# edwardyehuang/iSeg

Hardware: AMD Instinct MI355X
Metric: train_images_per_sec (ConvNeXt-T+ASPP 512x512 crop, fwd+bwd+AdamW, whole job) (higher is better)
Workload: dtype bf16

## Files before the change

### include/iseg_hip.h

```cpp
#ifndef ISEG_HIP_H
#define ISEG_HIP_H

#include <stddef.h>
#include <stdint.h>

#ifdef __cplusplus
extern "C" {
#endif

#ifndef ISEG_HIP_STREAM_T
#define ISEG_HIP_STREAM_T
typedef struct ihipStream_t* iseg_stream_t;
#endif

#define ISEG_STATUS_OK 0
#define ISEG_STATUS_ARG (-1)
#define ISEG_STATUS_HIP (-2)
#define ISEG_STATUS_UNSUPPORTED (-3)
#define ISEG_STATUS_WORKSPACE (-4)

#define ISEG_DTYPE_F32 0
#define ISEG_DTYPE_BF16 1

#define ISEG_ACT_NONE 0
#define ISEG_ACT_RELU 1
#define ISEG_ACT_GELU 2
#define ISEG_ACT_GELU_GRAD 3
#define ISEG_ACT_RELU_GRAD 4
#define ISEG_ACT_MUL_AUX 5
#define ISEG_ACT_SIGMOID 6
#define ISEG_ACT_SWISH 7

int iseg_version(void);
size_t iseg_last_error(char* buf_h, size_t n);

typedef struct iseg_gemm_args {
    const void* A;
    int64_t lda;
    int a_kcontig;
    const void* B;
    int64_t ldb;
    int b_kcontig;
    void* D;
    int64_t ldd;
    int64_t M, N, K;
    int in_dtype, out_dtype;
    const float* bias;
    const float* colscale;
    const float* rowscale;
    int64_t rows_per_group;
    const void* residual;
    int64_t ldr;
    const void* aux;
    int64_t ldaux;
    void* pre_out;
    int64_t ldp;
    int act;
    float alpha;
    int accumulate;
    int split_k;
    int a_act;
    float* colsum_out;
    int colsum_accumulate;
    int defer_reduce;
    int batch, batch_inner;
    int64_t sa_outer, sa_inner, sb_outer, sb_inner, sd_outer, sd_inner;
    int pre_deriv;
    int64_t b_group_rows, b_group_stride;
} iseg_gemm_args;

int iseg_gemm_splits(const iseg_gemm_args* args_h);
int iseg_gemm_slabs(const iseg_gemm_args* args_h);
int iseg_gemm_variant(const iseg_gemm_args* args_h);
size_t iseg_gemm_workspace_bytes(const iseg_gemm_args* args_h);
int iseg_gemm(const iseg_gemm_args* args_h, void* ws, size_t ws_bytes, iseg_stream_t stream);
int iseg_gemm_reduce(const iseg_gemm_args* args_h, void* ws, size_t ws_bytes, iseg_stream_t stream);
int iseg_gemm_tn_pair_splits(const iseg_gemm_args* g0, const iseg_gemm_args* g1);
int iseg_gemm_tn_pair(const iseg_gemm_args* g0, void* ws0, size_t ws0_bytes, const iseg_gemm_args* g1, void* ws1, size_t ws1_bytes,
                      iseg_stream_t stream);

int iseg_layernorm_fwd(const void* x, const float* gamma, const float* beta, void* y, float* mean, float* rstd, int64_t rows,
                       int C, float eps, int dtype, iseg_stream_t stream);
size_t iseg_layernorm_bwd_workspace_bytes(int64_t rows, int C);
int iseg_layernorm_bwd(const void* dy, const void* x, const float* gamma, const float* mean, const float* rstd, void* dx,
                       const void* dx_add, float* dgamma, float* dbeta, int accumulate_param_grads, int64_t rows, int C,
                       int dtype, void* ws, size_t ws_bytes, iseg_stream_t stream);
int iseg_layernorm_post_fwd(const void* x, const float* gamma, const float* beta, const float* colscale, const float* rowscale,
                            int64_t rows_per_group, const void* residual, void* y, float* mean, float* rstd, int64_t rows, int C, float eps,
                            int dtype, iseg_stream_t stream);
int iseg_layernorm_post_bwd(const void* dy, const void* x, const float* gamma, const float* beta, const float* colscale, const float* rowscale,
                            int64_t rows_per_group, const float* mean, const float* rstd, void* dx, float* dgamma, float* dbeta,
                            float* dcolscale, int64_t rows, int C, int dtype, void* ws, size_t ws_bytes, iseg_stream_t stream);
int iseg_layernorm_gather_fwd(const void* x, const int32_t* src_index, const float* gamma, const float* beta, void* y, float* mean,
                              float* rstd, int64_t rows_out, int C, float eps, int dtype, iseg_stream_t stream);
int iseg_layernorm_gather_bwd(const void* dy, const int32_t* dy_index, const void* x, const float* gamma, const float* mean,
                              const float* rstd, void* dx, const void* dx_add, float* dgamma, float* dbeta, int accumulate_param_grads,
                              int64_t rows, int C, int dtype, void* ws, size_t ws_bytes, iseg_stream_t stream);

int iseg_dwconv2d_fwd(const void* x, const float* w, const float* bias, const void* add, void* y, int N, int H, int W, int C,
                      int K, int dil, int pad_t, int pad_l, int flip, int dtype, iseg_stream_t stream);
int iseg_dwconv2d7_mfma(const void* x, const float* w, const float* bias, const void* add, void* y, int N, int H, int W, int C, int pad_t,
                        int pad_l, int flip, iseg_stream_t stream);
size_t iseg_dwconv2d_bwd_weight_workspace_bytes(int N, int H, int W, int C, int K);
int iseg_dwconv2d_bwd_weight(const void* x, const void* dy, float* dw, float* db, int accumulate, int N, int H, int W, int C,
                             int K, int dil, int pad_t, int pad_l, int dtype, void* ws, size_t ws_bytes, iseg_stream_t stream);

int iseg_dwconv2d_strided_fwd(const void* x, const float* w, const float* bias, void* y, int N, int H, int W, int C, int K, int stride, int dil,
                              int pad_t, int pad_l, int Ho, int Wo, int dtype, iseg_stream_t stream);
int iseg_dwconv2d_strided_bwd_data(const void* dy, const float* w, void* dx, int N, int H, int W, int C, int K, int stride, int dil, int pad_t,
                                   int pad_l, int Ho, int Wo, int dtype, iseg_stream_t stream);
size_t iseg_dwconv2d_strided_bwd_weight_workspace_bytes(int N, int Ho, int Wo, int C, int K);
int iseg_dwconv2d_strided_bwd_weight(const void* x, const void* dy, float* dw, float* db, int accumulate, int N, int H, int W, int C, int K,
                                     int stride, int dil, int pad_t, int pad_l, int Ho, int Wo, int dtype, void* ws, size_t ws_bytes,
                                     iseg_stream_t stream);

size_t iseg_bn_workspace_bytes(int64_t rows, int C);
int iseg_bn_stats(const void* x, int64_t ldx, float* packed, int64_t rows, int C, int dtype, void* ws, size_t ws_bytes,
                  iseg_stream_t stream);
int iseg_bn_finalize(const float* packed, int C, float eps, float momentum, float* mean, float* rstd, float* moving_mean,
                     float* moving_var, iseg_stream_t stream);
int iseg_bn_apply_fwd(const void* x, int64_t ldx, const float* mean, const float* rstd, const float* gamma, const float* beta,
                      void* y, int64_t ldy, int64_t rows, int C, int relu, int dtype, iseg_stream_t stream);
int iseg_bn_apply_fwd_packed(const void* x, int64_t ldx, const float* packed, float eps, float momentum, const float* gamma, const float* beta,
                             float* mean, float* rstd, float* moving_mean, float* moving_var, void* y, int64_t ldy, int64_t rows, int C,
                             int relu, int dtype, iseg_stream_t stream);
int iseg_bn_bwd_reduce(const void* dy, int64_t lddy, const void* x, int64_t ldx, const void* y, int64_t ldy, const float* mean,
                       const float* rstd, float* sums, int64_t rows, int C, int relu, int dtype, void* ws, size_t ws_bytes,
                       iseg_stream_t stream);
int iseg_bn_bwd_apply(const void* dy, int64_t lddy, const void* x, int64_t ldx, const void* y, int64_t ldy, const float* mean,
                      const float* rstd, const float* gamma, const float* sums, float inv_n, void* dx, int64_t lddx, int64_t rows,
                      int C, int relu, int dtype, iseg_stream_t stream);
int iseg_bn_bwd_apply_acc(const void* dy, int64_t lddy, const void* x, int64_t ldx, const void* y, int64_t ldy, const float* mean,
                          const float* rstd, const float* gamma, const float* sums, float inv_n, void* dx, int64_t lddx, float* dgamma,
                          float* dbeta, int64_t rows, int C, int relu, int dtype, iseg_stream_t stream);
int iseg_bn_bwd_reduce_remask(const void* dy, int64_t lddy, const void* x, int64_t ldx, const float* mean, const float* rstd,
                              const float* gamma, const float* beta, float* sums, int64_t rows, int C, int dtype, void* ws, size_t ws_bytes,
                              iseg_stream_t stream);
int iseg_bn_bwd_apply_remask(const void* dy, int64_t lddy, const void* x, int64_t ldx, const float* mean, const float* rstd,
                             const float* gamma, const float* beta, const float* sums, float inv_n, void* dx, int64_t lddx, float* dgamma,
                             float* dbeta, int64_t rows, int C, int dtype, iseg_stream_t stream);
int iseg_bn_relu_upsample_add(const void* z, const float* mean, const float* rstd, const float* gamma, const float* beta, const void* x,
                              void* out, int N, int Hi, int Wi, int Ho, int Wo, int C, int dtype, iseg_stream_t stream);
int iseg_rsqrt_eps(const float* var, float eps, float* out, int n, iseg_stream_t stream);

int iseg_mbconv_supported(int N, int HW, int C, int Cse);
size_t iseg_mbconv_partials_bytes(int N, int HW, int C, int backward);
size_t iseg_se_excite_bwd_workspace_bytes(int N, int C, int Cse);
int iseg_bn_swish_se_squeeze(const void* x, const float* mean, const float* rstd, const float* gamma, const float* beta, float* partials,
                             size_t partials_bytes, int N, int HW, int C, int dtype, iseg_stream_t stream);
int iseg_se_excite_fwd(const float* partials, int N, int HW, int C, int Cse, const float* W1, const float* b1, const float* W2, const float* b2,
                       float* m, float* hpre, float* g, iseg_stream_t stream);
int iseg_bn_swish_gate_fwd(const void* x, const float* mean, const float* rstd, const float* gamma, const float* beta, const float* g, void* out,
                           int N, int HW, int C, int dtype, iseg_stream_t stream);
int iseg_bn_swish_gate_bwd_reduce(const void* dO, const void* x, const float* mean, const float* rstd, const float* gamma, const float* beta,
                                  float* partials, size_t partials_bytes, int N, int HW, int C, int dtype, iseg_stream_t stream);
int iseg_se_excite_bwd(const float* partials, int N, int HW, int C, int Cse, const float* W1, const float* W2, const float* m, const float* hpre,
                       const float* g, float* dW1, float* db1, float* dW2, float* db2, int accumulate, float* dmh, float* sums, void* ws,
                       size_t ws_bytes, iseg_stream_t stream);
int iseg_bn_swish_gate_bwd_apply(const void* dO, const void* x, const float* mean, const float* rstd, const float* gamma, const float* beta,
                                 const float* g, const float* dmh, const float* sums, float inv_n, int train, void* dx, float* dgamma,
                                 float* dbeta, int N, int HW, int C, int dtype, iseg_stream_t stream);

int iseg_sepconv_supported(int N, int H, int W, int C, int stride, int dil, int dtype);
size_t iseg_relu_dwconv3_stats_workspace_bytes(int N, int H, int W, int C, int stride, int dil);
int iseg_relu_dwconv3_stats(const void* x, const float* w, void* z, float* packed, int N, int H, int W, int C, int stride, int dil, int dtype,
                            void* ws, size_t ws_bytes, iseg_stream_t stream);
int iseg_sepconv_fold(const float* W, const float* mean, const float* rstd, const float* gamma, const float* beta, void* Wt, void* Wn, float* bias,
                      int Cin, int Cout, int dtype, iseg_stream_t stream);
int iseg_sepconv_fold_bwd(const float* G, const float* S, const float* W, const float* mean, const float* rstd, const float* gamma,
                          const float* beta, float* dW, float* sums, float* dgamma, float* dbeta, int Cin, int Cout, iseg_stream_t stream);
size_t iseg_bnfold_dwconv3_relu_bwd_workspace_bytes(int N, int H, int W, int C, int stride, int dil);
int iseg_bnfold_dwconv3_relu_bwd(const void* D, const void* z, const void* x, const float* w, const float* mean, const float* rstd,
                                 const float* gamma, const float* sums, float inv_n, int train, void* dx, float* dw, int N, int H, int W, int C,
                                 int stride, int dil, int dtype, void* ws, size_t ws_bytes, iseg_stream_t stream);

int iseg_resblock_tail_supported(int C, int stride, int dtype);
size_t iseg_resblock_tail_workspace_bytes(int N, int H, int W, int C, int stride, int bn0);
int iseg_resblock_tail_fwd(const void* z2, const float* mean2, const float* rstd2, const float* gamma2, const float* beta2, const void* sc,
                           const float* mean0, const float* rstd0, const float* gamma0, const float* beta0, void* out, int N, int H, int W, int C,
                           int stride, int dtype, iseg_stream_t stream);
int iseg_resblock_tail_bwd_reduce(const void* dout, const void* out, const void* z2, const float* mean2, const float* rstd2, const void* z0,
                                  const float* mean0, const float* rstd0, float* sums, int N, int H, int W, int C, int stride, int dtype, void* ws,
                                  size_t ws_bytes, iseg_stream_t stream);
int iseg_resblock_tail_bwd_apply(const void* dout, const void* out, const void* z2, const float* mean2, const float* rstd2, const float* gamma2,
                                 const void* z0, const float* mean0, const float* rstd0, const float* gamma0, const float* sums, float inv_n2,
                                 float inv_n0, int train, void* dz2, void* dsc, float* dgamma2, float* dbeta2, float* dgamma0, float* dbeta0,
                                 int N, int H, int W, int C, int stride, int dtype, iseg_stream_t stream);

typedef void* iseg_comm_t;
int iseg_comm_unique_id(void* id128);
int iseg_comm_init(iseg_comm_t* comm, int world_size, int rank, const void* id128);
int iseg_allreduce_sum(iseg_comm_t comm, void* buf, size_t count, int dtype, iseg_stream_t stream);
int iseg_comm_destroy(iseg_comm_t comm);

int iseg_deferred_begin(void* grad_base, size_t grad_bytes, void* arena, size_t arena_bytes, iseg_stream_t stream);
int iseg_deferred_flush(iseg_stream_t stream);
int iseg_deferred_end(iseg_stream_t stream);
int iseg_cast(const void* src, int src_dtype, void* dst, int dst_dtype, int64_t n, iseg_stream_t stream);
int iseg_transpose_batched(const void* src, void* dst, const int64_t* table, int count, int max_tiles, iseg_stream_t stream);
int iseg_scale_cols_cast(const float* src, const float* colscale, void* dst, int64_t rows, int cols, int dst_dtype,
                         iseg_stream_t stream);
int iseg_im2col(const void* x, int in_dtype, void* col, int out_dtype, int N, int H, int W, int C, int KH, int KW, int sh, int sw,
                int dh, int dw, int pt, int pl, int Ho, int Wo, int64_t ldc, iseg_stream_t stream);
int iseg_col2im(const void* dcol, void* dx, int N, int H, int W, int C, int KH, int KW, int sh, int sw, int dh, int dw, int pt,
                int pl, int Ho, int Wo, int64_t ldc, int dtype, iseg_stream_t stream);
size_t iseg_colsum_workspace_bytes(int batch, int64_t rows, int C);
int iseg_colsum(const void* x, int64_t ldx, int64_t batch_stride, int batch, int64_t rows, int C, float* out, float scale,
                int accumulate, int dtype, void* ws, size_t ws_bytes, iseg_stream_t stream);
int iseg_broadcast_rows(const void* v, int v_dtype, void* y, int64_t ldy, int64_t batch_stride, int batch, int64_t rows, int C,
                        float scale, int accumulate, int dtype, iseg_stream_t stream);
int iseg_axpby(const void* a, const void* b, void* y, float alpha, float beta, int64_t n, int dtype, iseg_stream_t stream);
int iseg_accumulate_pair(const float* src, int n, float* dst0, float* dst1, iseg_stream_t stream);
int iseg_scale_dev(const void* x, const float* s_dev, void* y, int64_t n, int dtype, iseg_stream_t stream);
int iseg_rowscale(const void* x, const float* s, void* y, int64_t rows, int C, int64_t rows_per_group, int dtype,
                  iseg_stream_t stream);
int iseg_dropout(const void* x, void* y, int64_t n, float rate, uint64_t seed, const uint64_t* seed_offset, int dtype, iseg_stream_t stream);
int iseg_drop_path_mask(float* s, int n, float keep_prob, uint64_t seed, const uint64_t* seed_offset, iseg_stream_t stream);
int iseg_drop_path_masks(float* s, const float* keep_probs, int P, int n, uint64_t seed, const uint64_t* seed_offset, iseg_stream_t stream);
int iseg_fill_f32(float* p, float value, int64_t n, iseg_stream_t stream);
int iseg_dcnv2_sample_fwd(const void* x, const void* offset, void* col, int N, int H, int W, int C, int dtype, iseg_stream_t stream);
size_t iseg_dcnv2_sample_bwd_workspace_bytes(int N, int H, int W, int C);
// ... 263 lines not shown
```

### iseg_amd/_hip.py

```python
import ctypes as C
import os

_HERE = os.path.dirname(os.path.abspath(__file__))
LIB_PATH = os.path.join(_HERE, "lib", "libiseg_hip.so")

F32, BF16 = 0, 1
ACT_NONE, ACT_RELU, ACT_GELU, ACT_GELU_GRAD, ACT_RELU_GRAD, ACT_MUL_AUX, ACT_SIGMOID, ACT_SWISH = 0, 1, 2, 3, 4, 5, 6, 7


class HipLibraryMissing(RuntimeError):
    pass


class HipCallError(RuntimeError):
    pass


class GemmArgs(C.Structure):
    _fields_ = [
        ("A", C.c_void_p), ("lda", C.c_int64), ("a_kcontig", C.c_int),
        ("B", C.c_void_p), ("ldb", C.c_int64), ("b_kcontig", C.c_int),
        ("D", C.c_void_p), ("ldd", C.c_int64),
        ("M", C.c_int64), ("N", C.c_int64), ("K", C.c_int64),
        ("in_dtype", C.c_int), ("out_dtype", C.c_int),
        ("bias", C.c_void_p), ("colscale", C.c_void_p), ("rowscale", C.c_void_p), ("rows_per_group", C.c_int64),
        ("residual", C.c_void_p), ("ldr", C.c_int64),
        ("aux", C.c_void_p), ("ldaux", C.c_int64),
        ("pre_out", C.c_void_p), ("ldp", C.c_int64),
        ("act", C.c_int), ("alpha", C.c_float), ("accumulate", C.c_int), ("split_k", C.c_int), ("a_act", C.c_int),
        ("colsum_out", C.c_void_p), ("colsum_accumulate", C.c_int), ("defer_reduce", C.c_int),
        ("batch", C.c_int), ("batch_inner", C.c_int),
        ("sa_outer", C.c_int64), ("sa_inner", C.c_int64), ("sb_outer", C.c_int64), ("sb_inner", C.c_int64),
        ("sd_outer", C.c_int64), ("sd_inner", C.c_int64),
        ("pre_deriv", C.c_int),
        ("b_group_rows", C.c_int64),
        ("b_group_stride", C.c_int64),
    ]


class ConvGeom(C.Structure):
    _fields_ = [(n, C.c_int) for n in ("N", "H", "W", "Cin", "Cout", "KH", "KW", "sh", "sw", "dh", "dw", "pt", "pl", "Ho", "Wo", "groups")]


_p, _i, _l, _f, _z, _u64 = C.c_void_p, C.c_int, C.c_int64, C.c_float, C.c_size_t, C.c_uint64

SIGNATURES = {
    "iseg_version": (_i, []),
    "iseg_last_error": (_z, [C.c_char_p, _z]),
    "iseg_gemm_splits": (_i, [C.POINTER(GemmArgs)]),
    "iseg_gemm_tn_pair_splits": (_i, [C.POINTER(GemmArgs), C.POINTER(GemmArgs)]),
    "iseg_gemm_tn_pair": (_i, [C.POINTER(GemmArgs), _p, _z, C.POINTER(GemmArgs), _p, _z, _p]),
    "iseg_gemm_slabs": (_i, [C.POINTER(GemmArgs)]),
    "iseg_gemm_variant": (_i, [C.POINTER(GemmArgs)]),
    "iseg_gemm_workspace_bytes": (_z, [C.POINTER(GemmArgs)]),
    "iseg_gemm": (_i, [C.POINTER(GemmArgs), _p, _z, _p]),
    "iseg_gemm_reduce": (_i, [C.POINTER(GemmArgs), _p, _z, _p]),
    "iseg_layernorm_fwd": (_i, [_p, _p, _p, _p, _p, _p, _l, _i, _f, _i, _p]),
    "iseg_layernorm_bwd_workspace_bytes": (_z, [_l, _i]),
    "iseg_layernorm_bwd": (_i, [_p, _p, _p, _p, _p, _p, _p, _p, _p, _i, _l, _i, _i, _p, _z, _p]),
    "iseg_layernorm_post_fwd": (_i, [_p, _p, _p, _p, _p, _l, _p, _p, _p, _p, _l, _i, _f, _i, _p]),
    "iseg_layernorm_post_bwd": (_i, [_p, _p, _p, _p, _p, _p, _l, _p, _p, _p, _p, _p, _p, _l, _i, _i, _p, _z, _p]),
    "iseg_layernorm_gather_fwd": (_i, [_p, _p, _p, _p, _p, _p, _p, _l, _i, _f, _i, _p]),
    "iseg_layernorm_gather_bwd": (_i, [_p, _p, _p, _p, _p, _p, _p, _p, _p, _p, _i, _l, _i, _i, _p, _z, _p]),
    "iseg_dwconv2d_fwd": (_i, [_p, _p, _p, _p, _p, _i, _i, _i, _i, _i, _i, _i, _i, _i, _i, _p]),
    "iseg_dcnv2_sample_fwd": (_i, [_p, _p, _p, _i, _i, _i, _i, _i, _p]),
    "iseg_dcnv2_sample_bwd_workspace_bytes": (_z, [_i, _i, _i, _i]),
    "iseg_dcnv2_sample_bwd": (_i, [_p, _p, _p, _p, _p, _i, _i, _i, _i, _i, _p, _z, _p]),
    "iseg_qkv_rope": (_i, [_p, _p, _p, _p, _p, _l, _i, _i, _i, _i, _i, _i, _p]),
    "iseg_glu_fwd": (_i, [_p, _l, _p, _l, _p, _l, _l, _i, _i, _i, _p]),
    "iseg_glu_bwd": (_i, [_p, _l, _p, _l, _p, _l, _p, _l, _p, _l, _l, _i, _i, _i, _p]),
    "iseg_dwconv2d7_mfma": (_i, [_p, _p, _p, _p, _p, _i, _i, _i, _i, _i, _i, _i, _p]),
    "iseg_dwconv2d_bwd_weight_workspace_bytes": (_z, [_i, _i, _i, _i, _i]),
    "iseg_dwconv2d_bwd_weight": (_i, [_p, _p, _p, _p, _i, _i, _i, _i, _i, _i, _i, _i, _i, _i, _p, _z, _p]),
    "iseg_dwconv2d_strided_fwd": (_i, [_p, _p, _p, _p, _i, _i, _i, _i, _i, _i, _i, _i, _i, _i, _i, _i, _p]),
    "iseg_dwconv2d_strided_bwd_data": (_i, [_p, _p, _p, _i, _i, _i, _i, _i, _i, _i, _i, _i, _i, _i, _i, _p]),
    "iseg_dwconv2d_strided_bwd_weight_workspace_bytes": (_z, [_i, _i, _i, _i, _i]),
    "iseg_dwconv2d_strided_bwd_weight": (_i, [_p, _p, _p, _p, _i, _i, _i, _i, _i, _i, _i, _i, _i, _i, _i, _i, _i, _p, _z, _p]),
    "iseg_dcn_center_blend_fwd": (_i, [_p, _p, _p, _p, _l, _i, _i, _i, _p]),
    "iseg_dcn_center_blend_bwd": (_i, [_p, _p, _p, _p, _p, _p, _p, _l, _i, _i, _i, _p]),
    "iseg_bn_workspace_bytes": (_z, [_l, _i]),
    "iseg_bn_stats": (_i, [_p, _l, _p, _l, _i, _i, _p, _z, _p]),
    "iseg_bn_finalize": (_i, [_p, _i, _f, _f, _p, _p, _p, _p, _p]),
    "iseg_bn_apply_fwd": (_i, [_p, _l, _p, _p, _p, _p, _p, _l, _l, _i, _i, _i, _p]),
    "iseg_bn_apply_fwd_packed": (_i, [_p, _l, _p, _f, _f, _p, _p, _p, _p, _p, _p, _p, _l, _l, _i, _i, _i, _p]),
    "iseg_bn_bwd_reduce": (_i, [_p, _l, _p, _l, _p, _l, _p, _p, _p, _l, _i, _i, _i, _p, _z, _p]),
    "iseg_bn_bwd_apply": (_i, [_p, _l, _p, _l, _p, _l, _p, _p, _p, _p, _f, _p, _l, _l, _i, _i, _i, _p]),
    "iseg_bn_bwd_apply_acc": (_i, [_p, _l, _p, _l, _p, _l, _p, _p, _p, _p, _f, _p, _l, _p, _p, _l, _i, _i, _i, _p]),
    "iseg_bn_bwd_reduce_remask": (_i, [_p, _l, _p, _l, _p, _p, _p, _p, _p, _l, _i, _i, _p, _z, _p]),
    "iseg_bn_bwd_apply_remask": (_i, [_p, _l, _p, _l, _p, _p, _p, _p, _p, _f, _p, _l, _p, _p, _l, _i, _i, _p]),
    "iseg_bn_relu_upsample_add": (_i, [_p, _p, _p, _p, _p, _p, _p, _i, _i, _i, _i, _i, _i, _i, _p]),
    "iseg_rsqrt_eps": (_i, [_p, _f, _p, _i, _p]),
    "iseg_mbconv_supported": (_i, [_i, _i, _i, _i]),
    "iseg_mbconv_partials_bytes": (_z, [_i, _i, _i, _i]),
    "iseg_se_excite_bwd_workspace_bytes": (_z, [_i, _i, _i]),
    "iseg_bn_swish_se_squeeze": (_i, [_p, _p, _p, _p, _p, _p, _z, _i, _i, _i, _i, _p]),
    "iseg_se_excite_fwd": (_i, [_p, _i, _i, _i, _i, _p, _p, _p, _p, _p, _p, _p, _p]),
    "iseg_bn_swish_gate_fwd": (_i, [_p, _p, _p, _p, _p, _p, _p, _i, _i, _i, _i, _p]),
    "iseg_bn_swish_gate_bwd_reduce": (_i, [_p, _p, _p, _p, _p, _p, _p, _z, _i, _i, _i, _i, _p]),
    "iseg_se_excite_bwd": (_i, [_p, _i, _i, _i, _i, _p, _p, _p, _p, _p, _p, _p, _p, _p, _i, _p, _p, _p, _z, _p]),
    "iseg_bn_swish_gate_bwd_apply": (_i, [_p, _p, _p, _p, _p, _p, _p, _p, _p, _f, _i, _p, _p, _p, _i, _i, _i, _i, _p]),
    "iseg_sepconv_supported": (_i, [_i, _i, _i, _i, _i, _i, _i]),
    "iseg_relu_dwconv3_stats_workspace_bytes": (_z, [_i, _i, _i, _i, _i, _i]),
    "iseg_relu_dwconv3_stats": (_i, [_p, _p, _p, _p, _i, _i, _i, _i, _i, _i, _i, _p, _z, _p]),
    "iseg_sepconv_fold": (_i, [_p, _p, _p, _p, _p, _p, _p, _p, _i, _i, _i, _p]),
    "iseg_sepconv_fold_bwd": (_i, [_p, _p, _p, _p, _p, _p, _p, _p, _p, _p, _p, _i, _i, _p]),
    "iseg_bnfold_dwconv3_relu_bwd_workspace_bytes": (_z, [_i, _i, _i, _i, _i, _i]),
    "iseg_bnfold_dwconv3_relu_bwd": (_i, [_p, _p, _p, _p, _p, _p, _p, _p, _f, _i, _p, _p, _i, _i, _i, _i, _i, _i, _i, _p, _z, _p]),
    "iseg_resblock_tail_supported": (_i, [_i, _i, _i]),
    "iseg_resblock_tail_workspace_bytes": (_z, [_i, _i, _i, _i, _i, _i]),
    "iseg_resblock_tail_fwd": (_i, [_p, _p, _p, _p, _p, _p, _p, _p, _p, _p, _p, _i, _i, _i, _i, _i, _i, _p]),
    "iseg_resblock_tail_bwd_reduce": (_i, [_p, _p, _p, _p, _p, _p, _p, _p, _p, _i, _i, _i, _i, _i, _i, _p, _z, _p]),
    "iseg_resblock_tail_bwd_apply": (_i, [_p, _p, _p, _p, _p, _p, _p, _p, _p, _p, _p, _f, _f, _i, _p, _p, _p, _p, _p, _p, _i, _i, _i, _i, _i, _i, _p]),
    "iseg_cast": (_i, [_p, _i, _p, _i, _l, _p]),
    "iseg_deferred_begin": (_i, [_p, _z, _p, _z, _p]),
    "iseg_deferred_flush": (_i, [_p]),
    "iseg_deferred_end": (_i, [_p]),
    "iseg_transpose_batched": (_i, [_p, _p, _p, _i, _i, _p]),
    "iseg_scale_cols_cast": (_i, [_p, _p, _p, _l, _i, _i, _p]),
    "iseg_im2col": (_i, [_p, _i, _p, _i] + [_i] * 14 + [_l, _p]),
    "iseg_col2im": (_i, [_p, _p] + [_i] * 14 + [_l, _i, _p]),
    "iseg_colsum_workspace_bytes": (_z, [_i, _l, _i]),
    "iseg_colsum": (_i, [_p, _l, _l, _i, _l, _i, _p, _f, _i, _i, _p, _z, _p]),
    "iseg_broadcast_rows": (_i, [_p, _i, _p, _l, _l, _i, _l, _i, _f, _i, _i, _p]),
    "iseg_comm_unique_id": (_i, [_p]),
    "iseg_comm_init": (_i, [C.POINTER(C.c_void_p), _i, _i, _p]),
    "iseg_allreduce_sum": (_i, [_p, _p, _z, _i, _p]),
    "iseg_comm_destroy": (_i, [_p]),
    "iseg_axpby": (_i, [_p, _p, _p, _f, _f, _l, _i, _p]),
    "iseg_accumulate_pair": (_i, [_p, _i, _p, _p, _p]),
    "iseg_scale_dev": (_i, [_p, _p, _p, _l, _i, _p]),
    "iseg_rowscale": (_i, [_p, _p, _p, _l, _i, _l, _i, _p]),
    "iseg_dropout": (_i, [_p, _p, _l, _f, _u64, _p, _i, _p]),
    "iseg_drop_path_mask": (_i, [_p, _i, _f, _u64, _p, _p]),
    "iseg_drop_path_masks": (_i, [_p, _p, _i, _i, _u64, _p, _p]),
    "iseg_fill_f32": (_i, [_p, _f, _l, _p]),
    "iseg_act_fwd": (_i, [_p, _p, _l, _i, _i, _p]),
    "iseg_act_bwd": (_i, [_p, _p, _p, _l, _i, _i, _p]),
    "iseg_copy2d": (_i, [_p, _l, _p, _l, _l, _i, _i, _p]),
    "iseg_add2d_f32": (_i, [_p, _l, _p, _l, _l, _l, _p]),
    "iseg_scale_rows_f32": (_i, [_p, _p, _p, _l, _i, _p]),
    "iseg_layerscale_grads_workspace_bytes": (_z, [_i, _i]),
    "iseg_layerscale_grads": (_i, [_p, _p, _p, _p, _p, _p, _p, _p, _i, _i, _i, _p, _z, _p]),
    "iseg_layerscale_grads_slabs": (_i, [_p, _i, _p, _p, _p, _p, _p, _p, _i, _i, _i, _p, _z, _p]),
    "iseg_layerscale_grads_slabs_reduce": (_i, [_p, _i, _p, _p, _p, _p, _p, _p, _i, _i, _i, _p, _z, _p, _i, _l, _p, _p, _l, _i, _p]),
    "iseg_replace_nan_or_inf": (_i, [_p, _p, _l, _f, _i, _p, _z, _p]),
    "iseg_replace_nan_or_inf_bwd": (_i, [_p, _p, _p, _l, _i, _p]),
    "iseg_groupnorm_fwd": (_i, [_p, _p, _p, _p, _p, _p, _i, _i, _i, _i, _f, _i, _p]),
    "iseg_groupnorm_bwd_workspace_bytes": (_z, [_i, _i]),
    "iseg_groupnorm_bwd": (_i, [_p, _p, _p, _p, _p, _p, _p, _p, _i, _i, _i, _i, _i, _i, _p, _z, _p]),
    "iseg_rmsnorm_fwd": (_i, [_p, _p, _p, _p, _l, _i, _f, _i, _p]),
    "iseg_rmsnorm_bwd_workspace_bytes": (_z, [_l, _i]),
    "iseg_rmsnorm_bwd": (_i, [_p, _p, _p, _p, _p, _p, _i, _l, _i, _i, _p, _z, _p]),
    "iseg_grn_workspace_bytes": (_z, [_l, _l, _i]),
    "iseg_grn_fwd": (_i, [_p, _p, _p, _p, _p, _p, _l, _l, _i, _f, _i, _p, _z, _p]),
    "iseg_grn_bwd": (_i, [_p, _p, _p, _p, _p, _p, _p, _p, _p, _i, _l, _l, _i, _f, _i, _p, _z, _p]),
    "iseg_grn_fold_weights": (_i, [_p, _p, _p, _p, _l, _i, _i, _p]),
    "iseg_grn_fold_bias": (_i, [_p, _p, _p, _p, _i, _i, _p]),
    "iseg_grn_fold_wgrad": (_i, [_p, _i, _p, _p, _p, _p, _p, _p, _p, _i, _l, _i, _i, _p]),
    "iseg_grn_bwd_folded": (_i, [_p, _p, _p, _p, _p, _p, _p, _p, _p, _p, _i, _l, _l, _i, _f, _i, _p, _z, _p]),
    "iseg_softmax_rows_fwd": (_i, [_p, _p, _l, _i, _i, _i, _p, _i, _p, _i, _f, _f, _i, _p]),
    "iseg_softmax_rows_bwd": (_i, [_p, _p, _p, _l, _i, _i, _f, _f, _i, _p]),
    "iseg_clip_fwd": (_i, [_p, _p, _l, _f, _f, _i, _p]),
    "iseg_clip_bwd": (_i, [_p, _p, _p, _l, _f, _f, _i, _p]),
    "iseg_gather_rows": (_i, [_p, _p, _p, _l, _l, _i, _i, _p]),
    "iseg_gather_rows_fma": (_i, [_p, _p, _p, _l, _i, _p, _p, _l, _i, _i, _p]),
    "iseg_relpos_bias_scatter_grad_window": (_i, [_p, _i, _p, _i, _i, _i, _p]),
    "iseg_colsum_wide_workspace_bytes": (_z, [_l, _l]),
    "iseg_colsum_wide": (_i, [_p, _l, _l, _l, _p, _i, _i, _p, _z, _p]),
    "iseg_relpos_bias_gather": (_i, [_p, _p, _p, _i, _i, _p]),
    "iseg_relpos_bias_scatter_grad": (_i, [_p, _i, _p, _p, _i, _i, _i, _i, _p]),
    "iseg_dcnv3_fwd": (_i, [_p, _p, _p, _p] + [_i] * 10 + [_f, _i, _p]),
    "iseg_dcnv3_bwd_workspace_bytes": (_z, [_i] * 10 + [_f]),
    "iseg_dcnv3_bwd": (_i, [_p, _p, _p, _p, _p, _p, _p] + [_i] * 10 + [_f, _i, _p, _z, _p]),
    "iseg_dcnv3_fwd_ld": (_i, [_p, _p, _p, _l, _l, _p] + [_i] * 10 + [_f, _i, _p]),
    "iseg_dcnv3_bwd_side_bytes": (_z, [_i] * 10 + [_f]),
    "iseg_dcnv3_bwd_ld": (_i, [_p, _p, _p, _l, _l, _p, _p, _i, _p, _p] + [_i] * 10 + [_f, _i, _p, _z, _p, _z, _p]),
    "iseg_dcn_mask_softmax_fwd": (_i, [_p, _l, _i, _i, _l, _i, _i, _p]),
    "iseg_dcn_mask_softmax_bwd": (_i, [_p, _p, _l, _i, _i, _l, _i, _i, _p]),
    "iseg_split_cols_accumulate": (_i, [_p, _l, _l, _p, _i, _p, _i, _p]),
    "iseg_scale_cols": (_i, [_p, _p, _p, _l, _i, _i, _p]),
    "iseg_mul_colsum_workspace_bytes": (_z, [_l, _i]),
    "iseg_mul_colsum": (_i, [_p, _p, _l, _i, _p, _i, _i, _p, _z, _p]),
    "iseg_window_attention_supported": (_i, [_i, _i, _i]),
    "iseg_attention_fwd_supported": (_i, [_i, _i]),
    "iseg_attention_fwd": (_i, [_p, _p, _l, _i, _i, _i, _f, _i, _p]),
    "iseg_attention_lse_elems": (_z, [_l, _i, _i]),
    "iseg_attention_fwd_train": (_i, [_p, _p, _p, _l, _i, _i, _i, _f, _i, _p]),
    "iseg_attention_bwd_workspace_bytes": (_z, [_l, _i, _i]),
    "iseg_attention_bwd": (_i, [_p, _p, _p, _p, _p, _l, _i, _i, _i, _f, _i, _p, _z, _p]),
# ... 95 lines not shown
```

### iseg_amd/csrc/conv_igemm.hip

```cpp
#include <type_traits>

#include "gemm_impl.h"

using namespace iseg_mm;

int gemm_reduce(const iseg_gemm_args* g, const Epi& epi, float* slabs, int eff_split, int64_t slab_rows, hipStream_t stream);

namespace {

struct ConvP {
    const bf16_t* src;
    int Hs, Ws, Cs;
    int Hr, Wr;
    int Cg;
    int kw;
    int sh, sw, dh, dw, pt, pl;
    int groups;
};

struct PhaseP {
    int Hq, Wq;
    int a, b;
    int q0h, q0w;
    int Th, Tw;
    int tap0;
    int M, K;
};
constexpr int MAX_PHASES = 16;
struct PhaseTable {
    PhaseP ph[MAX_PHASES];
    int H, W, sh, sw, kw;
};
struct NoPhases {};

struct PhaseRows {
    int hw, wq, H, W, sh, sw, a, b;
    __device__ __forceinline__ int64_t operator()(int64_t m) const {
        const int n = (int)(m / hw), rem = (int)(m % hw);
        return ((int64_t)n * H + (rem / wq) * sh + a) * W + (rem % wq) * sw + b;
    }
};

constexpr int INVALID = -(1 << 28);

}

#include "conv_igemm_dma.h"

namespace {

__device__ __forceinline__ bf16x8 gather8(const ConvP& p, int nb, int ih, int iw, int c, bool ok) {
    bf16x8 v;
#pragma unroll
    for (int i = 0; i < 8; ++i) v[i] = (bf16_t)0.f;
    if (ok && ih >= 0 && ih < p.Hs && iw >= 0 && iw < p.Ws) v = *reinterpret_cast<const bf16x8*>(p.src + ((int64_t)(nb + ih * p.Ws + iw)) * p.Cs + c);
    return v;
}

template <int ROWS, int NT, int BK, int PASS> struct GatherStager : Stager<ROWS, PASS != 2, NT, BK> {
    using Base = Stager<ROWS, PASS != 2, NT, BK>;
    using G = typename Base::G;
    static constexpr int PT = Base::PER_THREAD;
    int a0[PT], a1[PT], a2[PT];

    __device__ __forceinline__ void prepare(const ConvP& p, int64_t row0, int64_t R, int coff, int tid) {
#pragma unroll
        for (int i = 0; i < PT; ++i) {
            const int c = tid + i * NT;
            int r, k;
            Base::decode(c, r, k);
            const int64_t row = row0 + r;
            a0[i] = INVALID;
            a1[i] = a2[i] = 0;
            if ((G::chunks % NT != 0 && c >= G::chunks) || row >= R) continue;
            if (PASS == 0) {
                const int hw = p.Hr * p.Wr, n = (int)(row / hw), rem = (int)(row % hw);
                a0[i] = (rem / p.Wr) * p.sh - p.pt;
                a1[i] = (rem % p.Wr) * p.sw - p.pl;
                a2[i] = n * p.Hs * p.Ws;
            } else if (PASS == 1) {
                const int hw = p.Hr * p.Wr, n = (int)(row / hw), rem = (int)(row % hw);
                a0[i] = rem / p.Wr + p.pt;
                a1[i] = rem % p.Wr + p.pl;
                a2[i] = n * p.Hs * p.Ws;
            } else {
                const int ij = (int)(row / p.Cg), ch = (int)(row % p.Cg);
                a0[i] = (ij / p.kw) * p.dh - p.pt;
                a1[i] = (ij % p.kw) * p.dw - p.pl;
                a2[i] = coff + ch;
            }
        }
    }
    __device__ __forceinline__ void gather(const ConvP& p, int64_t k0, int64_t Kend, int coff, int tid) {
#pragma unroll
        for (int i = 0; i < PT; ++i) {
            const int c = tid + i * NT;
            if (G::chunks % NT == 0 || c < G::chunks) {
                int r, k;
                Base::decode(c, r, k);
                const int kk = (int)(k0 + k);
                const bool ok = a0[i] != INVALID && kk < Kend;
                if (PASS == 0) {
                    const int ij = (int)(kk / p.Cg), ch = (int)(kk % p.Cg);
                    this->regs[i] = gather8(p, a2[i], a0[i] + (ij / p.kw) * p.dh, a1[i] + (ij % p.kw) * p.dw, coff + ch, ok);
                } else if (PASS == 1) {
                    const int ij = (int)(kk / p.Cg), ch = (int)(kk % p.Cg);
                    const int th = a0[i] - (ij / p.kw) * p.dh, tw = a1[i] - (ij % p.kw) * p.dw;
                    const bool hit = ok && th >= 0 && tw >= 0 && th % p.sh == 0 && tw % p.sw == 0;
                    this->regs[i] = gather8(p, a2[i], th / p.sh, tw / p.sw, coff + ch, hit);
                } else {
                    const int hw = p.Hr * p.Wr, n = (int)(kk / hw), rem = (int)(kk % hw);
                    this->regs[i] = gather8(p, n * p.Hs * p.Ws, (rem / p.Wr) * p.sh + a0[i], (rem % p.Wr) * p.sw + a1[i], a2[i], ok);
                }
            }
        }
    }
};

template <int ROWS, int NT, int BK> struct TapWeightStager : Stager<ROWS, true, NT, BK> {
    using Base = Stager<ROWS, true, NT, BK>;
    using G = typename Base::G;
    __device__ __forceinline__ void load_taps(const bf16_t* __restrict__ wg, int64_t ld, int64_t tap_stride, int cout_g, int64_t n0, int64_t k0,
                                              int64_t R, int64_t Kend, int tid, int tw, int tap0, int tsh, int tsw) {
#pragma unroll
        for (int i = 0; i < Base::PER_THREAD; ++i) {
            const int c = tid + i * NT;
            if (G::chunks % NT == 0 || c < G::chunks) {
                int r, k;
                Base::decode(c, r, k);
                const int kk = (int)(k0 + k);
                const int64_t row = n0 + r;
                bf16x8 v;
#pragma unroll
                for (int u = 0; u < 8; ++u) v[u] = (bf16_t)0.f;
                if (row < R && kk < Kend) {
                    const int ij = (int)(kk / cout_g), co = (int)(kk % cout_g);
                    const int tap = tap0 + (ij / tw) * tsh + (ij % tw) * tsw;
                    v = *reinterpret_cast<const bf16x8*>(wg + tap * tap_stride + row * ld + co);
                }
                this->regs[i] = v;
            }
        }
    }
};

template <int WM, int WN, int FM, int FN, int PASS, int BK, class TO>
__global__ __launch_bounds__(WM* WN * 64) void conv_igemm_kernel(ConvP p, const bf16_t* __restrict__ Bop, int64_t ldb, int64_t b_group_stride,
                                                                  int64_t tap_stride, TO* __restrict__ D, int64_t ldd, int64_t d_group_stride,
                                                                  int64_t M, int64_t N, int64_t K, int tiles_n, int ntiles,
                                                                  int64_t k_per_split, float* __restrict__ slabs, int64_t slab_group_stride,
                                                                  Epi epi, int vecD,
                                                                  typename std::conditional<PASS == 3, PhaseTable, NoPhases>::type phases) {
    constexpr bool AKC = PASS != 2, BKC = PASS == 1 || PASS == 3;
    constexpr int GPASS = PASS == 3 ? 1 : PASS;
    constexpr int NT = WM * WN * 64;
    constexpr int BM = WM * FM * 16, BN = WN * FN * 16;
    constexpr int TM = FM * 16, TN = FN * 16;
    constexpr int KS = BK / 32;
    using GA = TileGeom<BM, AKC, BK>;
    using GB = TileGeom<BN, BKC, BK>;
    constexpr int STAGE_ELEMS = GA::elems + GB::elems;
    constexpr int EPI_BYTES = WM * WN * 32 * (TN + 4) * 4;
    constexpr int LDS_BYTES = (STAGE_ELEMS * 2 > EPI_BYTES) ? STAGE_ELEMS * 2 : EPI_BYTES;
    __shared__ __attribute__((aligned(16))) char smem[LDS_BYTES];
    bf16_t* const lds = reinterpret_cast<bf16_t*>(smem);

    const int tid = threadIdx.x, lane = tid & 63, wid = tid >> 6;
    const int wm = wid / WN, wn = wid % WN;
    const int grp = blockIdx.z;
    const int coff = grp * p.Cg;
    Bop += grp * b_group_stride;
    D += grp * d_group_stride;
    if (slabs) slabs += grp * slab_group_stride;
    if (epi.bias) epi.bias += grp * N;

    int t, ksplit;
    int tw = p.kw, tap0 = 0, tsh = p.kw, tsw = 1;
    PhaseRows rows{};
    if constexpr (PASS == 3) {
        const PhaseP& ph = phases.ph[blockIdx.y];
        M = ph.M;
        K = ph.K;
        k_per_split = K;
        t = blockIdx.x;
        ksplit = 0;
        if ((int64_t)(t / tiles_n) * BM >= M) return;
        p.Hr = ph.Hq, p.Wr = ph.Wq, p.kw = ph.Tw, p.pt = ph.q0h, p.pl = ph.q0w;
        p.sh = p.sw = p.dh = p.dw = 1;
        tw = ph.Tw, tap0 = ph.tap0, tsh = phases.sh * phases.kw, tsw = phases.sw;
        rows = PhaseRows{ph.Hq * ph.Wq, ph.Wq, phases.H, phases.W, phases.sh, phases.sw, ph.a, ph.b};
    } else {
        tile_and_split(ntiles, t, ksplit);
    }
    const int tile_n = t % tiles_n, tile_m = t / tiles_n;
    const int64_t m0 = (int64_t)tile_m * BM, n0 = (int64_t)tile_n * BN;
    const int64_t kbeg = (int64_t)ksplit * k_per_split;
    const int64_t kend = (kbeg + k_per_split < K) ? kbeg + k_per_split : K;
    const int nk = (int)((kend - kbeg + BK - 1) / BK);

    f32x4 acc[FM][FN];
#pragma unroll
    for (int i = 0; i < FM; ++i)
#pragma unroll
        for (int j = 0; j < FN; ++j) acc[i][j] = f32x4{0.f, 0.f, 0.f, 0.f};

    GatherStager<BM, NT, BK, GPASS> sa;
    typename std::conditional<BKC, TapWeightStager<BN, NT, BK>, Stager<BN, false, NT, BK>>::type sb;
    sa.prepare(p, m0, M, coff, tid);

    auto load_b = [&](int64_t k0) {
        if constexpr (BKC) sb.load_taps(Bop, ldb, tap_stride, p.Cg, n0, k0, N, kend, tid, tw, tap0, tsh, tsw);
        else sb.load(Bop, ldb, n0, k0, N, kend, true, tid);
    };

    sa.gather(p, kbeg, kend, coff, tid);
    load_b(kbeg);
    sa.store(lds, tid);
    sb.store(lds + GA::elems, tid);
    __syncthreads();

    for (int kt = 0; kt < nk; ++kt) {
        const bool more = kt + 1 < nk;
        if (more) {
            const int64_t k0 = kbeg + (int64_t)(kt + 1) * BK;
            sa.gather(p, k0, kend, coff, tid);
            load_b(k0);
        }
#pragma unroll
        for (int ks = 0; ks < KS; ++ks) {
            bf16x8 af[FM], bfr[FN];
#pragma unroll
            for (int i = 0; i < FM; ++i) af[i] = read_frag<BM, AKC, BK>(lds, wm * TM + i * 16, ks, lane);
#pragma unroll
            for (int j = 0; j < FN; ++j) bfr[j] = read_frag<BN, BKC, BK>(lds + GA::elems, wn * TN + j * 16, ks, lane);
#pragma unroll
            for (int i = 0; i < FM; ++i)
#pragma unroll
                for (int j = 0; j < FN; ++j) acc[i][j] = __builtin_amdgcn_mfma_f32_16x16x32_bf16(bfr[j], af[i], acc[i][j], 0, 0, 0);
        }
        __syncthreads();
        if (more) {
            sa.store(lds, tid);
            sb.store(lds + GA::elems, tid);
            __syncthreads();
        }
    }
    if constexpr (PASS == 3) tile_epilogue<WM, WN, FM, FN, TO, PhaseRows>(acc, smem, D, ldd, M, N, m0, n0, wm, wn, wid, lane, nullptr, epi, false, vecD, 0, rows);
    else tile_epilogue<WM, WN, FM, FN, TO>(acc, smem, D, ldd, M, N, m0, n0, wm, wn, wid, lane, slabs, epi, false, vecD, ksplit);
}

struct Problem {
    int64_t M, N, K;
    ConvP p;
    const bf16_t* B;
    int64_t ldb, b_group_stride, tap_stride;
    void* D;
    int64_t ldd, d_group_stride;
    int out_dtype;
    const float* bias;
    int accumulate;
    int groups;
};

int conv_splits(int64_t M, int64_t N, int64_t K, int groups) {
    const int64_t tiles = ceil_div64(M, 128) * ceil_div64(N, N <= 64 ? 64 : 128) * groups;
    if (tiles >= 256 || K < 1024) return 1;
    int64_t want = 512 / tiles;
    const int64_t maxs = K / 512 > 0 ? K / 512 : 1;
    if (want > maxs) want = maxs;
    return (int)(want < 1 ? 1 : want);
}

template <int PASS, class TO> int run(const Problem& q, void* ws, size_t ws_bytes, hipStream_t stream, const char* what) {
    const int nsplit = q.groups > 1 ? 1 : conv_splits(q.M, q.N, q.K, 1);
    int64_t kps = q.K;
    float* slabs = nullptr;
    if (nsplit > 1) {
        const size_t need = (size_t)nsplit * q.groups * q.M * q.N * sizeof(float);
        if (!ws || ws_bytes < need) {
            iseg_set_error("%s: split-K needs %zu workspace bytes, got %zu", what, need, ws_bytes);
            return ISEG_ERR_WORKSPACE;
        }
        slabs = (float*)ws;
        kps = ceil_div64(ceil_div64(q.K, nsplit), 64) * 64;
    }
    const int eff = (int)ceil_div64(q.K, kps);
    Epi epi{};
    epi.bias = q.bias;
    epi.alpha = 1.f;
    epi.accumulate = q.accumulate;
    epi.batch_inner = 1;
    const int vecD = ((uintptr_t)q.D % 16 == 0) && (q.ldd % 8 == 0) && (q.d_group_stride % 8 == 0) && (!q.bias || (uintptr_t)q.bias % 16 == 0) &&
                     (q.N % 4 == 0);
    const int64_t slab_group_stride = 0;
    auto launch = [&](auto tile) {
        constexpr int WM = decltype(tile)::WM, WN = decltype(tile)::WN, FM = decltype(tile)::FM, FN = decltype(tile)::FN;
        constexpr int BM = WM * FM * 16, BN = WN * FN * 16;
        const int tiles_m = (int)ceil_div64(q.M, BM), tiles_n = (int)ceil_div64(q.N, BN);
        hipLaunchKernelGGL((conv_igemm_kernel<WM, WN, FM, FN, PASS, 64, TO>), dim3(tiles_m * tiles_n, eff, q.groups), dim3(WM * WN * 64), 0, stream, q.p,
                           q.B, q.ldb, q.b_group_stride, q.tap_stride, (TO*)q.D, q.ldd, q.d_group_stride, q.M, q.N, q.K, tiles_n, tiles_m * tiles_n,
                           kps, slabs, slab_group_stride, epi, vecD, NoPhases{});
    };
    struct T128 { enum { WM = 2, WN = 4, FM = 4, FN = 2 }; };
    struct T64 { enum { WM = 4, WN = 2, FM = 2, FN = 2 }; };
    if (q.N <= 64) launch(T64{});
    else launch(T128{});
    if (!slabs) return iseg_check_launch(what);
    iseg_gemm_args ga{};
    ga.M = q.M;
    ga.N = q.N;
    ga.K = q.K;
    ga.D = q.D;
    ga.ldd = q.ldd;
    ga.in_dtype = ISEG_BF16;
    ga.out_dtype = q.out_dtype;
    ga.alpha = 1.f;
    ga.accumulate = q.accumulate;
    ga.bias = q.bias;
    return gemm_reduce(&ga, epi, slabs, eff, q.M, stream);
}

int run_phases(const Problem& q, const iseg_conv_geom* g, hipStream_t stream, const char* what) {
    PhaseTable tab{};
    tab.H = g->H, tab.W = g->W, tab.sh = g->sh, tab.sw = g->sw, tab.kw = g->KW;
    const int og = g->Cout / g->groups;
    int count = 0;
    int64_t maxM = 0;
// ... 239 lines not shown
```

### iseg_amd/csrc/conv_igemm_dma.h

```cpp
#pragma once
#include "gemm_dma.h"

namespace {

__device__ uint4 conv_zero_page[8];

template <int WM, int WN, int NS, int PASS, class TO>
__global__ __launch_bounds__(WM* WN * 64) void conv_igemm_dma_kernel(ConvP p, const bf16_t* __restrict__ Bop, int64_t ldb, int64_t tap_stride,
                                                                      TO* __restrict__ D, int64_t ldd, int64_t M, int64_t N, int64_t K,
                                                                      int tiles_n, int ntiles, int64_t k_per_split, float* __restrict__ slabs,
                                                                      Epi epi) {
    using namespace iseg_mm;
    constexpr int FN = 4;
    constexpr int NW = WM * WN;
    constexpr int BM = WM * 64, BN = WN * FN * 16;
    constexpr int PIECES = (BM + BN) / 8, PPW = PIECES / NW;
    static_assert(PIECES % NW == 0, "stage pieces must divide over the wavefronts");
    constexpr int STAGE = (BM + BN) * 128;
    extern __shared__ __attribute__((aligned(1024))) char smem[];

    const int tid = threadIdx.x, lane = tid & 63, wid = tid >> 6;
    const int wm = wid / WN, wn = wid % WN;
    int t, ksplit;
    tile_and_split(ntiles, t, ksplit);
    const int64_t m0 = (int64_t)(t / tiles_n) * BM, n0 = (int64_t)(t % tiles_n) * BN;
    const int64_t kbeg = (int64_t)ksplit * k_per_split;
    const int64_t kend = (kbeg + k_per_split < K) ? kbeg + k_per_split : K;
    const int nk = (int)((kend - kbeg) / 64);

    int a0[PPW], a1[PPW];
    int64_t a2[PPW];
    const int rsub = lane >> 3;
    const bf16_t* const zero = reinterpret_cast<const bf16_t*>(conv_zero_page);
#pragma unroll
    for (int q = 0; q < PPW; ++q) {
        const int r = (wid + q * NW) * 8 + rsub;
        if (r < BM) {
            int64_t row = m0 + r;
            row = row < M ? row : M - 1;
            const int hw = p.Hr * p.Wr, n = (int)(row / hw), rem = (int)(row % hw);
            if (PASS == 0) {
                a0[q] = (rem / p.Wr) * p.sh - p.pt;
                a1[q] = (rem % p.Wr) * p.sw - p.pl;
            } else {
                a0[q] = rem / p.Wr + p.pt;
                a1[q] = rem % p.Wr + p.pl;
            }
            a2[q] = (int64_t)n * p.Hs * p.Ws;
        } else {
            const int rb = r - BM;
            int64_t row = n0 + rb;
            row = row < N ? row : N - 1;
            a0[q] = ((lane & 7) ^ b_key(rb)) * 8;
            a1[q] = 0;
            a2[q] = row * ldb;
        }
    }
    auto issue = [&](int stage, int kt) {
        const int64_t k0 = kbeg + (int64_t)kt * 64;
        const int tap = (int)(k0 / p.Cg), c0 = (int)(k0 % p.Cg);
        const int ti = tap / p.kw, tj = tap % p.kw;
#pragma unroll
        for (int q = 0; q < PPW; ++q) {
            const int r = (wid + q * NW) * 8 + rsub;
            const bf16_t* src;
            if (r < BM) {
                const int chunk = ((lane & 7) ^ (r & 7)) * 8;
                int ih, iw;
                bool ok;
                if (PASS == 0) {
                    ih = a0[q] + ti * p.dh;
                    iw = a1[q] + tj * p.dw;
                    ok = (unsigned)ih < (unsigned)p.Hs && (unsigned)iw < (unsigned)p.Ws;
                } else {
                    const int th = a0[q] - ti * p.dh, tw = a1[q] - tj * p.dw;
                    ih = th / p.sh;
                    iw = tw / p.sw;
                    ok = th >= 0 && tw >= 0 && ih * p.sh == th && iw * p.sw == tw && ih < p.Hs && iw < p.Ws;
                }
                src = ok ? p.src + (a2[q] + (int64_t)ih * p.Ws + iw) * p.Cs + c0 + chunk : zero + chunk;
            } else if (PASS == 0) {
                src = Bop + a2[q] + k0 + a0[q];
            } else {
                src = Bop + (int64_t)tap * tap_stride + a2[q] + c0 + a0[q];
            }
            __builtin_amdgcn_global_load_lds((glb_void_ptr)src, (lds_void_ptr)(smem + stage * STAGE + (wid + q * NW) * 1024), 16, 0, 0);
        }
    };

    f32x4 acc[4][FN];
    const int g = lane >> 4, c15 = lane & 15;
    const int a_sw = (g ^ (lane & 7)) * 16;
    const int a_off = (wm * 64 + c15) * 128;
    const int b_row0 = wn * (FN * 16) + 8 * (c15 >> 2) + (c15 & 3);
    const int b_sw = (g ^ b_key(b_row0)) * 16;
    const int b_off = BM * 128 + b_row0 * 128;
    auto compute = [&](int stage) {
        const char* sa = smem + stage * STAGE + a_off;
        const char* sb = smem + stage * STAGE + b_off;
#pragma unroll
        for (int ks = 0; ks < 2; ++ks) {
            bf16x8 af[4], bfr[FN];
#pragma unroll
            for (int i = 0; i < 4; ++i) af[i] = *reinterpret_cast<const bf16x8*>(sa + i * 2048 + (a_sw ^ (ks * 64)));
#pragma unroll
            for (int j = 0; j < FN; ++j) bfr[j] = *reinterpret_cast<const bf16x8*>(sb + ((j >> 1) * 32 + (j & 1) * 4) * 128 + (b_sw ^ (ks * 64)));
#pragma unroll
            for (int i = 0; i < 4; ++i)
#pragma unroll
                for (int j = 0; j < FN; ++j) acc[i][j] = __builtin_amdgcn_mfma_f32_16x16x32_bf16(bfr[j], af[i], acc[i][j], 0, 0, 0);
        }
    };
#pragma unroll
    for (int i = 0; i < 4; ++i)
#pragma unroll
        for (int j = 0; j < FN; ++j) acc[i][j] = f32x4{0.f, 0.f, 0.f, 0.f};
    if (NS == 2) {
        issue(0, 0);
        for (int kt = 0; kt < nk; ++kt) {
            const int stage = kt & 1;
            if (kt + 1 < nk) {
                issue(stage ^ 1, kt + 1);
                asm volatile("s_waitcnt vmcnt(%0)" ::"n"(PPW) : "memory");
            } else {
                asm volatile("s_waitcnt vmcnt(0)" ::: "memory");
            }
            __builtin_amdgcn_s_barrier();
            asm volatile("" ::: "memory");
            compute(stage);
            asm volatile("s_waitcnt lgkmcnt(0)" ::: "memory");
            __builtin_amdgcn_s_barrier();
            asm volatile("" ::: "memory");
        }
    } else {
#pragma unroll
        for (int q = 0; q < NS - 1; ++q)
            if (q < nk) issue(q, q);
        int stage = 0, fill = (NS - 1) % NS;
        for (int kt = 0; kt < nk; ++kt) {
            const int ahead = nk - 1 - kt;
            if (ahead >= NS - 2) asm volatile("s_waitcnt vmcnt(%0)" ::"n"((NS - 2) * PPW) : "memory");
            else asm volatile("s_waitcnt vmcnt(0)" ::: "memory");
            asm volatile("s_waitcnt lgkmcnt(0)" ::: "memory");
            __builtin_amdgcn_s_barrier();
            asm volatile("" ::: "memory");
            if (kt + NS - 1 < nk) issue(fill, kt + NS - 1);
            compute(stage);
            stage = stage + 1 == NS ? 0 : stage + 1;
            fill = fill + 1 == NS ? 0 : fill + 1;
        }
    }
    const bool split = slabs != nullptr;
    float* const slab = split ? slabs + (int64_t)ksplit * M * N : nullptr;
#pragma unroll
    for (int i = 0; i < 4; ++i) {
        const int64_t m = m0 + wm * 64 + i * 16 + c15;
#pragma unroll
        for (int h = 0; h < FN / 2; ++h) {
            const int64_t n = n0 + wn * (FN * 16) + 32 * h + 8 * g;
            if (m < M && n < N) {
                float v[8];
#pragma unroll
                for (int u = 0; u < 8; ++u) v[u] = acc[i][2 * h + (u >> 2)][u & 3];
                if (split) {
                    float* dst = slab + m * N + n;
                    *reinterpret_cast<float4*>(dst) = *reinterpret_cast<const float4*>(v);
                    *reinterpret_cast<float4*>(dst + 4) = *reinterpret_cast<const float4*>(v + 4);
                } else {
                    EpiPrefetch<TO> pf;
                    pf.load(epi, m, n, D, ldd);
                    epi_finish8<TO>(epi, v, pf, m, n, D, ldd);
                }
            }
        }
    }
// ... 4 lines not shown
```

### iseg_amd/csrc/gemm.hip

```cpp
#include "common.h"
#include "iseg_hip.h"

#include "gemm_dma_tn.h"

using namespace iseg_mm;

#include <stdlib.h>
#include <map>
#include <mutex>
#include <string>
namespace {
struct GemmCensus {
    std::mutex mu;
    std::map<std::string, long> seen;
    ~GemmCensus() {
        for (const auto& kv : seen) fprintf(stderr, "[iseg_gemm] %6ld x %s\n", kv.second, kv.first.c_str());
    }
};
bool gemm_log_on() {
    static const bool v = [] { const char* e = getenv("ISEG_GEMM_LOG"); return e && atoi(e) != 0; }();
    return v;
}
void gemm_log(const iseg_gemm_args* g, int nsplit) {
    static GemmCensus census;
    char buf[256];
    snprintf(buf, sizeof buf, "%s %s->%s M=%lld N=%lld K=%lld batch=%d split=%d form=%d act=%d a_act=%d%s%s%s%s%s%s%s%s%s%s", g->a_kcontig ? (g->b_kcontig ? "NT" : "NN") : (g->b_kcontig ? "TT" : "TN"),
             g->in_dtype == ISEG_BF16 ? "bf16" : "f32", g->out_dtype == ISEG_BF16 ? "bf16" : "f32", (long long)g->M, (long long)g->N, (long long)g->K,
             g->batch > 1 ? g->batch : 1, nsplit, iseg_gemm_variant(g), g->act, g->a_act, g->bias ? " bias" : "", g->residual ? " residual" : "",
             g->aux ? " aux" : "", g->pre_out ? " pre_out" : "", g->colsum_out ? " colsum" : "", g->colscale ? " colscale" : "", g->rowscale ? " rowscale" : "",
             g->pre_deriv ? " pre_deriv" : "", g->accumulate ? " accumulate" : "", g->alpha != 1.f ? " alpha" : "");
    std::lock_guard<std::mutex> lock(census.mu);
    ++census.seen[buf];
}
}
namespace iseg_mm {
int dma_bk32() {
    static const int v = [] {
        const char* e = getenv("ISEG_GEMM_DMA_BK32");
        return e ? atoi(e) : 1;
    }();
    return v;
}
}

namespace {

template <class TO>
__global__ __launch_bounds__(256) void gemm_f32_kernel(const float* __restrict__ A, int64_t sam, int64_t sak,
                                                       const float* __restrict__ B, int64_t sbk, int64_t sbn,
                                                       TO* __restrict__ D, int64_t ldd, int64_t M, int64_t N, int64_t K,
                                                       int tiles_n, int64_t k_per_split, float* __restrict__ slabs, Epi epi,
                                                       int a_act) {
    constexpr int TB = 64, TK = 16;
    __shared__ float sA[TK][TB + 1];
    __shared__ float sB[TK][TB + 1];
    const int tid = threadIdx.x;
    const int tx = tid & 15, ty = tid >> 4;
    if (gridDim.z > 1) {
        A += epi.off_a(blockIdx.z);
        B += epi.off_b(blockIdx.z);
        D += epi.off_d(blockIdx.z);
    }
    const int tile_n = blockIdx.x % tiles_n, tile_m = blockIdx.x / tiles_n;
    const int64_t m0 = (int64_t)tile_m * TB, n0 = (int64_t)tile_n * TB;
    const int64_t kbeg = (int64_t)blockIdx.y * k_per_split;
    const int64_t kend = (kbeg + k_per_split < K) ? kbeg + k_per_split : K;
    float acc[4][4] = {};
    for (int64_t k0 = kbeg; k0 < kend; k0 += TK) {
        for (int e = tid; e < TB * TK; e += 256) {
            int ka, ma;
            if (sak == 1) { ka = e % TK; ma = e / TK; } else { ma = e % TB; ka = e / TB; }
            const int64_t m = m0 + ma, k = k0 + ka;
            float av = (m < M && k < kend) ? A[m * sam + k * sak] : 0.f;
            if (a_act == ISEG_ACT_GELU) av = gelu_erf(av);
            sA[ka][ma] = av;
            int kb, nb;
            if (sbk == 1) { kb = e % TK; nb = e / TK; } else { nb = e % TB; kb = e / TB; }
            const int64_t n = n0 + nb, k2 = k0 + kb;
            sB[kb][nb] = (n < N && k2 < kend) ? B[k2 * sbk + n * sbn] : 0.f;
        }
        __syncthreads();
#pragma unroll
        for (int kk = 0; kk < TK; ++kk) {
            float a[4], b[4];
#pragma unroll
            for (int i = 0; i < 4; ++i) a[i] = sA[kk][ty * 4 + i];
#pragma unroll
            for (int j = 0; j < 4; ++j) b[j] = sB[kk][tx * 4 + j];
#pragma unroll
            for (int i = 0; i < 4; ++i)
#pragma unroll
                for (int j = 0; j < 4; ++j) acc[i][j] = fmaf(a[i], b[j], acc[i][j]);
        }
        __syncthreads();
    }
    const bool split = slabs != nullptr;
    for (int i = 0; i < 4; ++i)
        for (int j = 0; j < 4; ++j) {
            const int64_t m = m0 + ty * 4 + i, n = n0 + tx * 4 + j;
            if (m >= M || n >= N) continue;
            if (split) slabs[(int64_t)blockIdx.y * M * N + m * N + n] = acc[i][j];
            else D[m * ldd + n] = from_f32<TO>(epi_apply<TO>(epi, acc[i][j], m, n, D, ldd));
        }
}

template <class TO>
__global__ void splitk_reduce_kernel(const float* __restrict__ slabs, int nsplit, TO* __restrict__ D, int64_t ldd, int64_t M,
                                     int64_t N, Epi epi, int64_t slab_rows) {
    const int64_t total = slab_rows * N;
    for (int64_t i = blockIdx.x * (int64_t)blockDim.x + threadIdx.x; i < total; i += (int64_t)gridDim.x * blockDim.x) {
        float s = 0.f;
        for (int z = 0; z < nsplit; ++z) s += slabs[(int64_t)z * total + i];
        const int64_t m = i / N, n = i % N;
        if (m < M) D[m * ldd + n] = from_f32<TO>(epi_apply<TO>(epi, s, m, n, D, ldd));
        else epi.colsum_out[n] = s + (epi.colsum_accumulate ? epi.colsum_out[n] : 0.f);
    }
}

int choose_split(const iseg_gemm_args* g, int tile) {
    if (g->split_k > 0) return g->split_k;
    if (const int form = iseg_mm::dma_tn_form(g)) {
        const int s = iseg_mm::dma_tn_split(g, form);
        if (s > 1) return s;
    }
    const int64_t tiles = ceil_div64(g->M + (g->colsum_out ? 1 : 0), tile) * ceil_div64(g->N, tile);
    if (tiles >= 256 || g->K < 2048 || g->batch > 1 || g->b_group_rows > 0) return 1;
    if (g->in_dtype == ISEG_BF16 && tiles >= 96 && iseg_mm::dma_eligible(g, 128)) return 1;
    int64_t want = 512 / tiles;
    if (want < 1) want = 1;
    const int64_t maxs = g->K / 512 > 0 ? g->K / 512 : 1;
    if (want > maxs) want = maxs;
    if (want > 512) want = 512;
    return (int)(want < 1 ? 1 : want);
}

}

int gemm_reduce(const iseg_gemm_args* g, const Epi& epi, float* slabs, int eff_split, int64_t slab_rows, hipStream_t stream);

extern "C" int iseg_gemm_splits(const iseg_gemm_args* g) {
    return choose_split(g, g->in_dtype == ISEG_BF16 ? 128 : 64);
}

extern "C" int iseg_gemm_slabs(const iseg_gemm_args* g) {
    if (!g) return 0;
    const int nsplit = iseg_gemm_splits(g);
    if (nsplit <= 1) return 1;
    const int64_t kps = ceil_div64(ceil_div64(g->K, nsplit), 128) * 128;
    return (int)ceil_div64(g->K, kps);
}

extern "C" int iseg_gemm_variant(const iseg_gemm_args* g) {
    if (!g || g->in_dtype != ISEG_BF16) return 0;
    const int nsplit = iseg_gemm_splits(g);
    const int64_t kps = nsplit > 1 ? ceil_div64(ceil_div64(g->K, nsplit), 128) * 128 : g->K;
    if (nsplit > 1 && iseg_mm::dma_tn_form(g)) return iseg_mm::dma_tn_form(g);
    if (!iseg_mm::dma_eligible(g, kps)) return 0;
    return iseg_mm::dma_form(g, (int)ceil_div64(g->K, kps));
}

extern "C" size_t iseg_gemm_workspace_bytes(const iseg_gemm_args* g) {
    const int s = iseg_gemm_splits(g);
    return s > 1 ? (size_t)s * (size_t)(g->M + (g->colsum_out ? 1 : 0)) * (size_t)g->N * sizeof(float) : 0;
}

extern "C" int iseg_gemm(const iseg_gemm_args* g, void* ws, size_t ws_bytes, hipStream_t stream) {
    ISEG_REQUIRE(g && g->A && g->B && g->D, "iseg_gemm: null operand");
    ISEG_REQUIRE(g->M > 0 && g->N > 0 && g->K > 0, "iseg_gemm: empty problem M=%lld N=%lld K=%lld", (long long)g->M,
                 (long long)g->N, (long long)g->K);
    ISEG_REQUIRE(g->in_dtype == ISEG_F32 || g->in_dtype == ISEG_BF16, "iseg_gemm: bad in_dtype %d", g->in_dtype);
    ISEG_REQUIRE(g->out_dtype == ISEG_F32 || g->out_dtype == ISEG_BF16, "iseg_gemm: bad out_dtype %d", g->out_dtype);
    ISEG_REQUIRE(!(g->in_dtype == ISEG_F32 && g->out_dtype == ISEG_BF16), "iseg_gemm: f32 inputs need f32 output");
    ISEG_REQUIRE(!g->rowscale || g->rows_per_group > 0, "iseg_gemm: rowscale needs rows_per_group");
    ISEG_REQUIRE((g->act != ISEG_ACT_GELU_GRAD && g->act != ISEG_ACT_RELU_GRAD && g->act != ISEG_ACT_MUL_AUX) || g->aux,
                 "iseg_gemm: act needs aux");
    ISEG_REQUIRE(g->act >= ISEG_ACT_NONE && g->act <= ISEG_ACT_MUL_AUX, "iseg_gemm: bad act %d", g->act);
    ISEG_REQUIRE(!g->pre_deriv || (g->act == ISEG_ACT_GELU && g->pre_out), "iseg_gemm: pre_deriv needs act = GELU and pre_out");
    ISEG_REQUIRE(g->a_act == ISEG_ACT_NONE || g->a_act == ISEG_ACT_GELU, "iseg_gemm: a_act must be NONE or GELU");
    Epi epi{g->bias, g->colscale, g->rowscale, g->rows_per_group, g->residual, g->ldr, g->aux, g->ldaux, g->pre_out, g->ldp,
            g->act, g->alpha, g->accumulate, g->colsum_out, g->colsum_accumulate,
            g->batch_inner > 0 ? g->batch_inner : 1, g->sa_outer, g->sa_inner, g->sb_outer, g->sb_inner, g->sd_outer, g->sd_inner,
            g->pre_deriv, g->b_group_rows, g->b_group_stride};
    const int batch = g->batch > 1 ? g->batch : 1;
    if (batch > 1) {
        ISEG_REQUIRE(batch <= 65535, "iseg_gemm: batch %d exceeds the grid z limit (65535)", batch);
        ISEG_REQUIRE(!g->bias && !g->colscale && !g->rowscale && !g->residual && !g->aux && !g->pre_out && !g->colsum_out &&
                         g->act == ISEG_ACT_NONE && g->a_act == ISEG_ACT_NONE,
                     "iseg_gemm: a batched problem takes only the alpha / accumulate epilogue");
    }
    if (g->b_group_rows > 0) {
        if (!(g->in_dtype == ISEG_BF16 && g->a_kcontig && g->b_kcontig && batch == 1 && g->split_k <= 1 && g->b_group_rows % 256 == 0 &&
              g->b_group_stride % 8 == 0 && iseg_mm::dma_eligible(g, g->K))) {
            iseg_set_error("iseg_gemm: B per row group needs the LDS-DMA path (bf16, K-contiguous operands, K %% 64 == 0, aligned) with "
                           "b_group_rows %% 256 == 0, no split and no batch");
            return ISEG_ERR_UNSUPPORTED;
        }
    }
    if (g->colsum_out) {
        ISEG_REQUIRE(g->in_dtype == ISEG_BF16 && !g->a_kcontig && !g->b_kcontig, "iseg_gemm: colsum_out needs the bf16 wgrad orientation");
        ISEG_REQUIRE(g->M % 8 == 0, "iseg_gemm: colsum_out needs M %% 8 == 0");
    }
    const int64_t slab_rows = g->M + (g->colsum_out ? 1 : 0);
    const int nsplit = iseg_gemm_splits(g);
    if (gemm_log_on()) gemm_log(g, nsplit);
    float* slabs = nullptr;
    int64_t kps = g->K;
    if (nsplit > 1) {
        const size_t need = (size_t)nsplit * slab_rows * g->N * sizeof(float);
        if (!ws || ws_bytes < need) {
            iseg_set_error("iseg_gemm: split-K needs %zu workspace bytes, got %zu", need, ws_bytes);
            return ISEG_ERR_WORKSPACE;
        }
        slabs = (float*)ws;
        kps = ceil_div64(ceil_div64(g->K, nsplit), 128) * 128;
    }
    const int eff_split = (int)ceil_div64(g->K, kps);
    if (g->in_dtype == ISEG_BF16) {
        if (g->a_kcontig && !g->b_kcontig) gemm_bf16_nn(g, epi, eff_split, kps, slabs, stream);
        else if (g->a_kcontig && g->b_kcontig) gemm_bf16_nt(g, epi, eff_split, kps, slabs, stream);
        else if (!g->a_kcontig && !g->b_kcontig) gemm_bf16_tn(g, epi, eff_split, kps, slabs, stream);
        else {
            iseg_set_error("iseg_gemm: bf16 path does not provide A MN-contiguous x B K-contiguous");
            return ISEG_ERR_UNSUPPORTED;
        }
    } else {
        const int tiles_m = (int)ceil_div64(g->M, 64), tiles_n = (int)ceil_div64(g->N, 64);
        const int64_t sam = g->a_kcontig ? g->lda : 1, sak = g->a_kcontig ? 1 : g->lda;
        const int64_t sbk = g->b_kcontig ? 1 : g->ldb, sbn = g->b_kcontig ? g->ldb : 1;
        hipLaunchKernelGGL((gemm_f32_kernel<float>), dim3(tiles_m * tiles_n, eff_split, batch), dim3(256), 0, stream,
                           (const float*)g->A, sam, sak, (const float*)g->B, sbk, sbn, (float*)g->D, g->ldd, g->M, g->N, g->K,
                           tiles_n, kps, slabs, epi, g->a_act);
    }
    if (g->defer_reduce) return iseg_check_launch("iseg_gemm");
    return gemm_reduce(g, epi, slabs, eff_split, slab_rows, stream);
}

int gemm_reduce(const iseg_gemm_args* g, const Epi& epi, float* slabs, int eff_split, int64_t slab_rows, hipStream_t stream) {
    const bool plain_epilogue = !g->bias && !g->colscale && !g->rowscale && !g->residual && !g->pre_out && g->act == ISEG_ACT_NONE &&
                                g->out_dtype == ISEG_F32 && g->ldd == g->N &&
                                (!g->colsum_out || (g->colsum_accumulate != 0) == (g->accumulate != 0));
    if (slabs && plain_epilogue) {
        const int64_t mn = g->M * g->N;
        launch_reduce_rows(slabs, eff_split, slab_rows * g->N, 0, 1, slab_rows * g->N, (float*)g->D, g->colsum_out, mn, 0, g->alpha,
                           g->accumulate, stream);
        (void)mn;
    } else if (slabs) {
        const int64_t total = slab_rows * g->N;
        const int blocks = (int)(ceil_div64(total, 256) < 2048 ? ceil_div64(total, 256) : 2048);
        if (g->out_dtype == ISEG_BF16)
            hipLaunchKernelGGL((splitk_reduce_kernel<bf16_t>), dim3(blocks), dim3(256), 0, stream, slabs, eff_split,
                               (bf16_t*)g->D, g->ldd, g->M, g->N, epi, slab_rows);
        else
            hipLaunchKernelGGL((splitk_reduce_kernel<float>), dim3(blocks), dim3(256), 0, stream, slabs, eff_split,
                               (float*)g->D, g->ldd, g->M, g->N, epi, slab_rows);
    }
    return iseg_check_launch("iseg_gemm");
}

extern "C" int iseg_gemm_tn_pair_splits(const iseg_gemm_args* g0, const iseg_gemm_args* g1) {
    if (!g0 || !g1) return 0;
    iseg_gemm_args a = *g0, b = *g1;
    a.split_k = b.split_k = 0;
    return iseg_mm::gemm_bf16_tn_pair_split(&a, &b);
}

extern "C" int iseg_gemm_tn_pair(const iseg_gemm_args* g0, void* ws0, size_t ws0_bytes, const iseg_gemm_args* g1, void* ws1, size_t ws1_bytes,
                                 hipStream_t stream) {
    ISEG_REQUIRE(g0 && g1 && g0->A && g0->B && g1->A && g1->B, "iseg_gemm_tn_pair: null operand");
    const int s = iseg_gemm_tn_pair_splits(g0, g1);
    ISEG_REQUIRE(s > 1 && g0->split_k == s && g1->split_k == s, "iseg_gemm_tn_pair: the problems do not pair (splits %d, split_k %d / %d)", s, g0->split_k,
                 g1->split_k);
    ISEG_REQUIRE(!g0->bias && !g1->bias && g0->act == ISEG_ACT_NONE && g1->act == ISEG_ACT_NONE && g0->out_dtype == ISEG_F32 && g1->out_dtype == ISEG_F32,
                 "iseg_gemm_tn_pair: plain fp32 weight gradients only");
    const size_t need0 = iseg_gemm_workspace_bytes(g0), need1 = iseg_gemm_workspace_bytes(g1);
    if (!ws0 || ws0_bytes < need0 || !ws1 || ws1_bytes < need1) {
        iseg_set_error("iseg_gemm_tn_pair: needs %zu + %zu workspace bytes, got %zu + %zu", need0, need1, ws0_bytes, ws1_bytes);
        return ISEG_ERR_WORKSPACE;
    }
    const int64_t kps = ceil_div64(ceil_div64(g0->K, s), 128) * 128;
    const int eff = (int)ceil_div64(g0->K, kps);
    iseg_mm::gemm_bf16_tn_pair(g0, (float*)ws0, g1, (float*)ws1, eff, kps, stream);
    return iseg_check_launch("iseg_gemm_tn_pair");
}

extern "C" int iseg_gemm_reduce(const iseg_gemm_args* g, void* ws, size_t ws_bytes, hipStream_t stream) {
    ISEG_REQUIRE(g && g->D, "iseg_gemm_reduce: null argument");
    const int nsplit = iseg_gemm_splits(g);
    if (nsplit <= 1) return ISEG_OK;
    const int64_t slab_rows = g->M + (g->colsum_out ? 1 : 0);
    const size_t need = (size_t)nsplit * slab_rows * g->N * sizeof(float);
    if (!ws || ws_bytes < need) {
        iseg_set_error("iseg_gemm_reduce: needs %zu workspace bytes, got %zu", need, ws_bytes);
        return ISEG_ERR_WORKSPACE;
    }
    const int64_t kps = ceil_div64(ceil_div64(g->K, nsplit), 128) * 128;
    const int eff_split = (int)ceil_div64(g->K, kps);
    Epi epi{g->bias, g->colscale, g->rowscale, g->rows_per_group, g->residual, g->ldr, g->aux, g->ldaux, g->pre_out, g->ldp,
            g->act, g->alpha, g->accumulate, g->colsum_out, g->colsum_accumulate,
            g->batch_inner > 0 ? g->batch_inner : 1, g->sa_outer, g->sa_inner, g->sb_outer, g->sb_inner, g->sd_outer, g->sd_inner,
            g->pre_deriv, g->b_group_rows, g->b_group_stride};
    const int batch = g->batch > 1 ? g->batch : 1;
    if (batch > 1) {
        ISEG_REQUIRE(batch <= 65535, "iseg_gemm: batch %d exceeds the grid z limit (65535)", batch);
        ISEG_REQUIRE(!g->bias && !g->colscale && !g->rowscale && !g->residual && !g->aux && !g->pre_out && !g->colsum_out &&
                         g->act == ISEG_ACT_NONE && g->a_act == ISEG_ACT_NONE,
                     "iseg_gemm: a batched problem takes only the alpha / accumulate epilogue");
    }
    return gemm_reduce(g, epi, (float*)ws, eff_split, slab_rows, stream);
}
```

### iseg_amd/csrc/gemm_dma.h

```cpp
#pragma once
#include "gemm_impl.h"
#include <stdlib.h>

namespace iseg_mm {

typedef __attribute__((address_space(3))) void* lds_void_ptr;
typedef const __attribute__((address_space(1))) void* glb_void_ptr;

__device__ __forceinline__ int b_key(int row) { return (row & 3) | (((row >> 3) & 1) << 2); }

enum { EK_ANY = 0, EK_GELU_DERIV = 1, EK_MUL_AUX = 2, EK_BIAS_RESIDUAL = 3, EK_PLAIN = 4, EK_BIAS = 5 };

template <int EK> __device__ __forceinline__ Epi epi_known(Epi e) {
    if (EK == EK_GELU_DERIV) {
        e.act = ISEG_ACT_GELU;
        e.pre_deriv = 1;
        e.residual = nullptr;
        e.aux = nullptr;
        e.colscale = nullptr;
        e.accumulate = 0;
        e.alpha = 1.f;
    } else if (EK == EK_MUL_AUX) {
        e.act = ISEG_ACT_MUL_AUX;
        e.bias = nullptr;
        e.pre_out = nullptr;
        e.residual = nullptr;
        e.colscale = nullptr;
        e.accumulate = 0;
        e.alpha = 1.f;
    } else if (EK == EK_PLAIN) {
        e.act = ISEG_ACT_NONE;
        e.bias = nullptr;
        e.aux = nullptr;
        e.pre_out = nullptr;
        e.residual = nullptr;
        e.colscale = nullptr;
        e.rowscale = nullptr;
        e.accumulate = 0;
        e.alpha = 1.f;
    } else if (EK == EK_BIAS) {
        e.act = ISEG_ACT_NONE;
        e.aux = nullptr;
        e.pre_out = nullptr;
        e.residual = nullptr;
        e.colscale = nullptr;
        e.rowscale = nullptr;
        e.accumulate = 0;
        e.alpha = 1.f;
    } else if (EK == EK_BIAS_RESIDUAL) {
        e.act = ISEG_ACT_NONE;
        e.aux = nullptr;
        e.pre_out = nullptr;
        e.accumulate = 0;
        e.alpha = 1.f;
    }
    return e;
}

static __device__ __attribute__((aligned(16))) unsigned int dma_zero_chunk[4] = {0u, 0u, 0u, 0u};

constexpr int dma_min_k = 32;

inline int epi_kind(const Epi& e, const float* slabs) {
    if (slabs || e.alpha != 1.f || e.accumulate) return EK_ANY;
    if (e.act == ISEG_ACT_GELU && e.pre_out && e.pre_deriv && e.bias && !e.residual && !e.aux && !e.colscale) return EK_GELU_DERIV;
    if (e.act == ISEG_ACT_MUL_AUX && e.aux && !e.bias && !e.pre_out && !e.residual && !e.colscale) return EK_MUL_AUX;
    if (e.act == ISEG_ACT_NONE && e.bias && e.residual && !e.aux && !e.pre_out) return EK_BIAS_RESIDUAL;
    if (e.act == ISEG_ACT_NONE && e.bias && !e.residual && !e.aux && !e.pre_out && !e.colscale && !e.rowscale) return EK_BIAS;
    if (e.act == ISEG_ACT_NONE && !e.bias && !e.residual && !e.aux && !e.pre_out && !e.colscale && !e.rowscale) return EK_PLAIN;
    return EK_ANY;
}

__device__ __forceinline__ int key32(int quad) { return (0x6C >> (2 * (quad & 3))) & 3; }

template <int WM, int WN, int NS, class TO, int FN = 4, int EK = EK_ANY, bool KT = false, int BKS = 64, int FM = 4>
__global__ __launch_bounds__(WM* WN * 64) __attribute__((amdgpu_waves_per_eu(BKS == 32 ? 4 : 1, BKS == 32 ? 4 : 8))) void gemm_bf16_dma_kernel(const bf16_t* __restrict__ A, int64_t lda, const bf16_t* __restrict__ B,
                                                                     int64_t ldb, TO* __restrict__ D, int64_t ldd, int64_t M, int64_t N,
                                                                     int64_t K, int tiles_n, int ntiles, int64_t k_per_split,
                                                                     float* __restrict__ slabs, Epi epi, int vecD) {
    constexpr int NW = WM * WN;
    constexpr int BM = WM * FM * 16, BN = WN * FN * 16;
    static_assert(FN % 2 == 0, "column fragments come in pairs (eight consecutive columns per lane)");
    static_assert(BKS == 64 || (BKS == 32 && !KT), "ring stages hold 64 or 32 K elements; the 32 form has no K tail");
    constexpr int RB = BKS * 2;
    constexpr int CPR = BKS / 8;
    constexpr int RPP = 1024 / RB;
    constexpr int PIECES = (BM + BN) / RPP;
    constexpr int PPW = PIECES / NW;
    static_assert(PIECES % NW == 0, "stage pieces must divide over the wavefronts");
    constexpr int STAGE = (BM + BN) * RB;
    extern __shared__ __attribute__((aligned(1024))) char smem[];

    const int tid = threadIdx.x, lane = tid & 63, wid = tid >> 6;
    const int wm = wid / WN, wn = wid % WN;
    if (gridDim.z > 1) {
        A += epi.off_a(blockIdx.z);
        B += epi.off_b(blockIdx.z);
        D += epi.off_d(blockIdx.z);
    }
    int t, ksplit;
    tile_and_split(ntiles, t, ksplit);
    const int64_t m0 = (int64_t)(t / tiles_n) * BM, n0 = (int64_t)(t % tiles_n) * BN;
    const int64_t kbeg = (int64_t)ksplit * k_per_split;
    const int64_t kend = (kbeg + k_per_split < K) ? kbeg + k_per_split : K;
    const int nk = KT ? (int)((kend - kbeg + 63) / 64) : (int)((kend - kbeg) / BKS);
    const int tail_chunks = KT ? (int)(((kend - kbeg) & 63) >> 3) : 0;

    const bf16_t* src[PPW];
    bool beyond[PPW];
    auto point = [&](int64_t pm0, int64_t pn0) {
        const int rsub = lane / CPR;
#pragma unroll
        for (int p = 0; p < PPW; ++p) {
            const int r = (wid + p * NW) * RPP + rsub;
            if (r < BM) {
                int64_t row = pm0 + r;
                row = row < M ? row : M - 1;
                const int ch = (lane & (CPR - 1)) ^ (BKS == 64 ? (r & 7) : key32(r >> 2));
                src[p] = A + row * lda + kbeg + ch * 8;
                beyond[p] = ch >= tail_chunks;
            } else {
                const int rb = r - BM;
                int64_t row = pn0 + rb;
                row = row < N ? row : N - 1;
                const bf16_t* Bg = epi.b_group_rows > 0 ? B + (pm0 / epi.b_group_rows) * epi.b_group_stride : B;
                const int ch = (lane & (CPR - 1)) ^ (BKS == 64 ? b_key(rb) : key32(rb >> 3));
                src[p] = Bg + row * ldb + kbeg + ch * 8;
                beyond[p] = ch >= tail_chunks;
            }
        }
    };
    point(m0, n0);
    auto issue = [&](int stage, int kstep) {
        if (KT && tail_chunks != 0 && kstep == nk - 1) {
#pragma unroll
            for (int p = 0; p < PPW; ++p) {
                const bf16_t* s = beyond[p] ? reinterpret_cast<const bf16_t*>(dma_zero_chunk) : src[p];
                __builtin_amdgcn_global_load_lds((glb_void_ptr)s, (lds_void_ptr)(smem + stage * STAGE + (wid + p * NW) * 1024), 16, 0, 0);
                src[p] += 64;
            }
            return;
        }
#pragma unroll
        for (int p = 0; p < PPW; ++p) {
            __builtin_amdgcn_global_load_lds((glb_void_ptr)src[p], (lds_void_ptr)(smem + stage * STAGE + (wid + p * NW) * 1024), 16, 0, 0);
            src[p] += BKS;
        }
    };

    f32x4 acc[FM][FN];

    const int g = lane >> 4, c15 = lane & 15;
    const int a_sw = (BKS == 64 ? (g ^ (lane & 7)) : (g ^ key32(c15 >> 2))) * 16;
    const int a_off = (wm * (FM * 16) + c15) * RB;
    const int b_row0 = wn * (FN * 16) + 8 * (c15 >> 2) + (c15 & 3);
    const int b_sw = (BKS == 64 ? (g ^ b_key(b_row0)) : (g ^ key32(c15 >> 2))) * 16;
    const int b_off = BM * RB + b_row0 * RB;

    auto compute = [&](int stage) {
        const char* sa = smem + stage * STAGE + a_off;
        const char* sb = smem + stage * STAGE + b_off;
#pragma unroll
        for (int ks = 0; ks < BKS / 32; ++ks) {
            bf16x8 af[FM], bfr[FN];
#pragma unroll
            for (int i = 0; i < FM; ++i) af[i] = *reinterpret_cast<const bf16x8*>(sa + i * 16 * RB + (a_sw ^ (ks * 64)));
#pragma unroll
            for (int j = 0; j < FN; ++j) bfr[j] = *reinterpret_cast<const bf16x8*>(sb + ((j >> 1) * 32 + (j & 1) * 4) * RB + (b_sw ^ (ks * 64)));
#pragma unroll
            for (int i = 0; i < FM; ++i)
#pragma unroll
                for (int j = 0; j < FN; ++j) acc[i][j] = __builtin_amdgcn_mfma_f32_16x16x32_bf16(bfr[j], af[i], acc[i][j], 0, 0, 0);
        }
    };
#pragma unroll
    for (int i = 0; i < FM; ++i)
#pragma unroll
        for (int j = 0; j < FN; ++j) acc[i][j] = f32x4{0.f, 0.f, 0.f, 0.f};
    if (NS == 2) {
        issue(0, 0);
        for (int kt = 0; kt < nk; ++kt) {
            const int stage = kt & 1;
            if (kt + 1 < nk) {
                issue(stage ^ 1, kt + 1);
                asm volatile("s_waitcnt vmcnt(%0)" ::"n"(PPW) : "memory");
            } else {
                asm volatile("s_waitcnt vmcnt(0)" ::: "memory");
            }
            __builtin_amdgcn_s_barrier();
            asm volatile("" ::: "memory");
            compute(stage);
            asm volatile("s_waitcnt lgkmcnt(0)" ::: "memory");
            __builtin_amdgcn_s_barrier();
            asm volatile("" ::: "memory");
        }
    } else {
#pragma unroll
        for (int p = 0; p < NS - 1; ++p)
            if (p < nk) issue(p, p);
        int stage = 0, fill = (NS - 1) % NS;
        for (int kt = 0; kt < nk; ++kt) {
            const int ahead = nk - 1 - kt;
            if (ahead >= NS - 2) asm volatile("s_waitcnt vmcnt(%0)" ::"n"((NS - 2) * PPW) : "memory");
            else if (NS > 3 && ahead == 1) asm volatile("s_waitcnt vmcnt(%0)" ::"n"(PPW) : "memory");
            else asm volatile("s_waitcnt vmcnt(0)" ::: "memory");
            asm volatile("s_waitcnt lgkmcnt(0)" ::: "memory");
            __builtin_amdgcn_s_barrier();
            asm volatile("" ::: "memory");
            if (kt + NS - 1 < nk) issue(fill, kt + NS - 1);
            compute(stage);
            stage = stage + 1 == NS ? 0 : stage + 1;
            fill = fill + 1 == NS ? 0 : fill + 1;
        }
        asm volatile("s_waitcnt lgkmcnt(0)" ::: "memory");
        __builtin_amdgcn_s_barrier();
        asm volatile("" ::: "memory");
    }
    const bool split = slabs != nullptr;
    float* const slab = split ? slabs + (int64_t)ksplit * M * N : nullptr;
#pragma unroll
    for (int i = 0; i < FM; ++i) {
        const int64_t m = m0 + wm * (FM * 16) + i * 16 + c15;
#pragma unroll
        for (int h = 0; h < FN / 2; ++h) {
            const int64_t n = n0 + wn * (FN * 16) + 32 * h + 8 * g;
            if (m < M && n < N) {
                float v[8];
#pragma unroll
                for (int u = 0; u < 8; ++u) v[u] = acc[i][2 * h + (u >> 2)][u & 3];
                if (split) {
                    float* dst = slab + m * N + n;
                    *reinterpret_cast<float4*>(dst) = *reinterpret_cast<const float4*>(v);
                    *reinterpret_cast<float4*>(dst + 4) = *reinterpret_cast<const float4*>(v + 4);
                } else {
                    const Epi ek = epi_known<EK>(epi);
                    EpiPrefetch<TO> pf;
                    pf.load(ek, m, n, D, ldd);
                    epi_finish8<TO>(ek, v, pf, m, n, D, ldd);
                }
            }
        }
    }
}

inline bool dma_eligible(const iseg_gemm_args* g, int64_t kps) {
    if (!g->a_kcontig || !g->b_kcontig || g->a_act != ISEG_ACT_NONE || g->colsum_out) return false;
    if (g->K % 8 != 0 || (kps != g->K && kps % 64 != 0) || g->K < dma_min_k || g->N % 8 != 0 || g->N < 64 || g->M < 64) return false;
    if (((uintptr_t)g->A % 16) || ((uintptr_t)g->B % 16) || g->lda % 8 || g->ldb % 8) return false;
    if (((uintptr_t)g->D % 16) || g->ldd % 8) return false;
    if (g->residual && (((uintptr_t)g->residual % 16) || g->ldr % 8)) return false;
    if (g->aux && (((uintptr_t)g->aux % 16) || g->ldaux % 8)) return false;
    if (g->pre_out && (((uintptr_t)g->pre_out % 16) || g->ldp % 8)) return false;
    if ((g->bias && (uintptr_t)g->bias % 16) || (g->colscale && (uintptr_t)g->colscale % 16)) return false;
    if (g->batch > 1 && (g->sa_outer % 8 || g->sa_inner % 8 || g->sb_outer % 8 || g->sb_inner % 8 || g->sd_outer % 8 || g->sd_inner % 8))
        return false;
    return true;
}

template <int WM, int WN, int NS, class TO, int FN = 4, int EK = EK_ANY, int BKS = 64, int FM = 4>
void launch_dma(const iseg_gemm_args* g, const Epi& epi, int nsplit, int64_t k_per_split, float* slabs, hipStream_t s) {
    constexpr int BM = WM * FM * 16, BN = WN * FN * 16;
    const int tiles_m = (int)ceil_div64(g->M, BM), tiles_n = (int)ceil_div64(g->N, BN);
    const int ntiles = tiles_m * tiles_n;
    const int vecD = 1;
    const int batch = g->batch > 1 ? g->batch : 1;
    dim3 grid(ntiles, nsplit, batch);
    constexpr int lds = NS * (BM + BN) * BKS * 2;
    static_assert(FM == 4 || BKS == 64, "the 32-deep stages exist for the 256 x 128 tile");
    if constexpr (BKS == 32) {
        static const bool raised32 = [] {
            return hipFuncSetAttribute(reinterpret_cast<const void*>(&gemm_bf16_dma_kernel<WM, WN, NS, TO, FN, EK, false, 32>),
                                       hipFuncAttributeMaxDynamicSharedMemorySize, lds) == hipSuccess;
        }();
        (void)raised32;
        hipLaunchKernelGGL((gemm_bf16_dma_kernel<WM, WN, NS, TO, FN, EK, false, 32>), grid, dim3(WM * WN * 64), lds, s, (const bf16_t*)g->A, g->lda,
                           (const bf16_t*)g->B, g->ldb, (TO*)g->D, g->ldd, g->M, g->N, g->K, tiles_n, ntiles, k_per_split, slabs, epi, vecD);
        return;
    }
    if (g->K % 64 != 0) {
        static const bool raised_kt = [] {
            return hipFuncSetAttribute(reinterpret_cast<const void*>(&gemm_bf16_dma_kernel<WM, WN, NS, TO, FN, EK, true, 64, FM>),
                                       hipFuncAttributeMaxDynamicSharedMemorySize, lds) == hipSuccess;
        }();
        (void)raised_kt;
        hipLaunchKernelGGL((gemm_bf16_dma_kernel<WM, WN, NS, TO, FN, EK, true, 64, FM>), grid, dim3(WM * WN * 64), lds, s, (const bf16_t*)g->A, g->lda,
                           (const bf16_t*)g->B, g->ldb, (TO*)g->D, g->ldd, g->M, g->N, g->K, tiles_n, ntiles, k_per_split, slabs, epi, vecD);
        return;
    }
    static const bool raised = [] {
        return hipFuncSetAttribute(reinterpret_cast<const void*>(&gemm_bf16_dma_kernel<WM, WN, NS, TO, FN, EK, false, 64, FM>),
                                   hipFuncAttributeMaxDynamicSharedMemorySize, lds) == hipSuccess;
    }();
    (void)raised;
    hipLaunchKernelGGL((gemm_bf16_dma_kernel<WM, WN, NS, TO, FN, EK, false, 64, FM>), grid, dim3(WM * WN * 64), lds, s, (const bf16_t*)g->A, g->lda,
                       (const bf16_t*)g->B, g->ldb, (TO*)g->D, g->ldd, g->M, g->N, g->K, tiles_n, ntiles, k_per_split, slabs, epi, vecD);
}

inline int dma_variant(const iseg_gemm_args* g, int nsplit) {
    const int64_t tiles256 = ceil_div64(g->M, 256) * ceil_div64(g->N, 128), tiles128 = ceil_div64(g->M, 128) * ceil_div64(g->N, 128);
    if (g->N <= 64) return 1;
    if (tiles256 * nsplit >= 192) return 2;
    if (tiles128 * nsplit >= 384) return 3;
    return 4;
}

inline int dma_cus() {
    static const int n = [] {
        int dev = 0, v = 0;
        if (hipGetDevice(&dev) != hipSuccess || hipDeviceGetAttribute(&v, hipDeviceAttributeMultiprocessorCount, dev) != hipSuccess || v < 8) v = 256;
        return v;
    }();
    return n;
}

inline int dma_form(const iseg_gemm_args* g, int nsplit) {
    const int variant = dma_variant(g, nsplit);
    static const int flat = [] { const char* e = getenv("ISEG_GEMM_DMA_64X192"); return e ? atoi(e) : 1; }();
    if (flat && variant == 4 && nsplit == 1 && g->batch <= 1 && g->N % 192 == 0 && g->K % 64 == 0) {
        const int64_t t4 = ceil_div64(g->M, 128) * ceil_div64(g->N, 128), t9 = ceil_div64(g->M, 64) * (g->N / 192);
        if (t4 * 8 <= (int64_t)dma_cus() * 7 && t9 <= dma_cus() && t9 * 6 >= t4 * 7) return 9;
    }
    if (variant != 2 || nsplit != 1 || g->batch > 1) return variant;
    const int cus = dma_cus();
    const int64_t t128 = ceil_div64(g->M, 256) * ceil_div64(g->N, 128);
    static const int tall = [] { const char* e = getenv("ISEG_GEMM_DMA_128X192"); return e ? atoi(e) : 1; }();
    if (tall && g->N % 192 == 0 && t128 * 8 <= (int64_t)cus * 7) {
        const int64_t t8 = ceil_div64(g->M, 128) * (g->N / 192);
        if (t8 <= cus && t8 * 6 >= t128 * 7) return 8;
    }
    if (g->N % 192 == 0) {
        const int64_t t192 = ceil_div64(g->M, 256) * (g->N / 192);
        const double e128 = (double)t128 / (double)(ceil_div64(t128, cus) * cus), e192 = (double)t192 / (double)(ceil_div64(t192, cus) * cus);
        if (t192 >= cus && e192 >= e128 + 0.1) return 6;
    }
    return variant;
}

template <int WM, int WN, int NS, class TO, int FN, int BKS = 64, int FM = 4>
void launch_dma_kinds(const iseg_gemm_args* g, const Epi& epi, int nsplit, int64_t kps, float* slabs, hipStream_t s) {
    if (sizeof(TO) == 2) {
        switch (epi_kind(epi, slabs)) {
            case EK_GELU_DERIV: launch_dma<WM, WN, NS, TO, FN, EK_GELU_DERIV, BKS, FM>(g, epi, nsplit, kps, slabs, s); return;
            case EK_MUL_AUX: launch_dma<WM, WN, NS, TO, FN, EK_MUL_AUX, BKS, FM>(g, epi, nsplit, kps, slabs, s); return;
            case EK_BIAS_RESIDUAL: launch_dma<WM, WN, NS, TO, FN, EK_BIAS_RESIDUAL, BKS, FM>(g, epi, nsplit, kps, slabs, s); return;
            case EK_PLAIN: launch_dma<WM, WN, NS, TO, FN, EK_PLAIN, BKS, FM>(g, epi, nsplit, kps, slabs, s); return;
            case EK_BIAS: launch_dma<WM, WN, NS, TO, FN, EK_BIAS, BKS, FM>(g, epi, nsplit, kps, slabs, s); return;
            default: break;
        }
    }
    launch_dma<WM, WN, NS, TO, FN, EK_ANY, BKS, FM>(g, epi, nsplit, kps, slabs, s);
}

int dma_bk32();

template <class TO>
void dispatch_dma(const iseg_gemm_args* g, const Epi& epi, int nsplit, int64_t kps, float* slabs, hipStream_t s) {
    switch (dma_form(g, nsplit)) {
        case 1: launch_dma<2, 1, 4, TO>(g, epi, nsplit, kps, slabs, s); break;
        case 2:
            if (dma_bk32() && (dma_bk32() == 2 || g->K <= 512) && g->K % 32 == 0 && g->K >= 96 && (kps == g->K || kps % 64 == 0) && sizeof(TO) == 2)
                launch_dma_kinds<4, 2, 3, TO, 4, 32>(g, epi, nsplit, kps, slabs, s);
            else launch_dma_kinds<4, 2, 3, TO, 4>(g, epi, nsplit, kps, slabs, s);
            break;
        case 3: launch_dma<2, 2, 2, TO>(g, epi, nsplit, kps, slabs, s); break;
        case 6: launch_dma_kinds<4, 2, 2, TO, 6>(g, epi, nsplit, kps, slabs, s); break;
        case 9: launch_dma_kinds<4, 2, 3, TO, 6, 64, 1>(g, epi, nsplit, kps, slabs, s); break;
        case 8: launch_dma_kinds<4, 2, 3, TO, 6, 64, 2>(g, epi, nsplit, kps, slabs, s); break;
        default: launch_dma_kinds<2, 2, 3, TO, 4>(g, epi, nsplit, kps, slabs, s); break;
    }
}

}
```

### iseg_amd/csrc/gemm_impl.h

```cpp
#pragma once
#include "common.h"
#include "iseg_hip.h"

namespace iseg_mm {

struct Epi {
    const float* bias;
    const float* colscale;
    const float* rowscale;
    int64_t rows_per_group;
    const void* residual;
    int64_t ldr;
    const void* aux;
    int64_t ldaux;
    void* pre_out;
    int64_t ldp;
    int act;
    float alpha;
    int accumulate;
    float* colsum_out;
    int colsum_accumulate;
    int batch_inner;
    int64_t sa_outer, sa_inner, sb_outer, sb_inner, sd_outer, sd_inner;
    int pre_deriv;
    int64_t b_group_rows, b_group_stride;
    __device__ __forceinline__ int64_t off_a(int z) const { return (z / batch_inner) * sa_outer + (z % batch_inner) * sa_inner; }
    __device__ __forceinline__ int64_t off_b(int z) const { return (z / batch_inner) * sb_outer + (z % batch_inner) * sb_inner; }
    __device__ __forceinline__ int64_t off_d(int z) const { return (z / batch_inner) * sd_outer + (z % batch_inner) * sd_inner; }
};

template <class TO>
__device__ __forceinline__ float epi_apply(const Epi& e, float acc, int64_t m, int64_t n, const TO* D, int64_t ldd) {
    float v = acc * e.alpha;
    if (e.bias) v += e.bias[n];
    if (e.pre_out) reinterpret_cast<TO*>(e.pre_out)[m * e.ldp + n] = from_f32<TO>(e.pre_deriv ? gelu_erf_grad(v) : v);
    if (e.act == ISEG_ACT_RELU) v = fmaxf(v, 0.f);
    else if (e.act == ISEG_ACT_GELU) v = gelu_erf(v);
    else if (e.act == ISEG_ACT_GELU_GRAD) v *= gelu_erf_grad(to_f32(reinterpret_cast<const TO*>(e.aux)[m * e.ldaux + n]));
    else if (e.act == ISEG_ACT_RELU_GRAD) v = to_f32(reinterpret_cast<const TO*>(e.aux)[m * e.ldaux + n]) > 0.f ? v : 0.f;
    else if (e.act == ISEG_ACT_MUL_AUX) v *= to_f32(reinterpret_cast<const TO*>(e.aux)[m * e.ldaux + n]);
    if (e.colscale) v *= e.colscale[n];
    if (e.rowscale) v *= e.rowscale[m / e.rows_per_group];
    if (e.residual) v += to_f32(reinterpret_cast<const TO*>(e.residual)[m * e.ldr + n]);
    if (e.accumulate) v += to_f32(D[m * ldd + n]);
    return v;
}

template <class TO>
__device__ __forceinline__ void epi_apply8(const Epi& e, float* v, int64_t m, int64_t n, TO* D, int64_t ldd) {
#pragma unroll
    for (int i = 0; i < 8; ++i) v[i] *= e.alpha;
    if (e.bias) {
        float b[8];
        load8<float>(e.bias + n, b);
#pragma unroll
        for (int i = 0; i < 8; ++i) v[i] += b[i];
    }
    constexpr bool FAST = sizeof(TO) == 2;
    if (e.pre_out && !e.pre_deriv) store8<TO>(reinterpret_cast<TO*>(e.pre_out) + m * e.ldp + n, v);
    if (e.act == ISEG_ACT_RELU) {
#pragma unroll
        for (int i = 0; i < 8; ++i) v[i] = fmaxf(v[i], 0.f);
    } else if (e.act == ISEG_ACT_GELU) {
        if (e.pre_out && e.pre_deriv) {
            float d[8];
#pragma unroll
            for (int i = 0; i < 8; ++i) {
                if (FAST) gelu_sig_both(v[i], v[i], d[i]);
                else {
                    d[i] = gelu_erf_grad(v[i]);
                    v[i] = gelu_erf(v[i]);
                }
            }
            store8<TO>(reinterpret_cast<TO*>(e.pre_out) + m * e.ldp + n, d);
        } else {
#pragma unroll
            for (int i = 0; i < 8; ++i) v[i] = FAST ? gelu_poly(v[i]) : gelu_erf(v[i]);
        }
    } else if (e.act == ISEG_ACT_MUL_AUX) {
        float a[8];
        load8<TO>(reinterpret_cast<const TO*>(e.aux) + m * e.ldaux + n, a);
#pragma unroll
        for (int i = 0; i < 8; ++i) v[i] *= a[i];
    } else if (e.act == ISEG_ACT_GELU_GRAD) {
        float a[8];
        load8<TO>(reinterpret_cast<const TO*>(e.aux) + m * e.ldaux + n, a);
#pragma unroll
        for (int i = 0; i < 8; ++i) v[i] *= FAST ? gelu_poly_grad(a[i]) : gelu_erf_grad(a[i]);
    } else if (e.act == ISEG_ACT_RELU_GRAD) {
        float a[8];
        load8<TO>(reinterpret_cast<const TO*>(e.aux) + m * e.ldaux + n, a);
#pragma unroll
        for (int i = 0; i < 8; ++i) v[i] = a[i] > 0.f ? v[i] : 0.f;
    }
    if (e.colscale) {
        float c[8];
        load8<float>(e.colscale + n, c);
#pragma unroll
        for (int i = 0; i < 8; ++i) v[i] *= c[i];
    }
    if (e.rowscale) {
        const float s = e.rowscale[m / e.rows_per_group];
#pragma unroll
        for (int i = 0; i < 8; ++i) v[i] *= s;
    }
    if (e.residual) {
        float r[8];
        load8<TO>(reinterpret_cast<const TO*>(e.residual) + m * e.ldr + n, r);
#pragma unroll
        for (int i = 0; i < 8; ++i) v[i] += r[i];
    }
    if (e.accumulate) {
        float r[8];
        load8<TO>(D + m * ldd + n, r);
#pragma unroll
        for (int i = 0; i < 8; ++i) v[i] += r[i];
    }
    store8<TO>(D + m * ldd + n, v);
}

template <class T> struct Raw8;
template <> struct Raw8<bf16_t> {
    bf16x8 v;
    __device__ __forceinline__ void load(const bf16_t* p) { v = *reinterpret_cast<const bf16x8*>(p); }
    __device__ __forceinline__ float get(int i) const { return (float)v[i]; }
};
template <> struct Raw8<float> {
    float4 a, b;
    __device__ __forceinline__ void load(const float* p) {
        a = *reinterpret_cast<const float4*>(p);
        b = *reinterpret_cast<const float4*>(p + 4);
    }
    __device__ __forceinline__ float get(int i) const {
        return i == 0 ? a.x : i == 1 ? a.y : i == 2 ? a.z : i == 3 ? a.w : i == 4 ? b.x : i == 5 ? b.y : i == 6 ? b.z : b.w;
    }
};

template <class TO> struct EpiPrefetch {
    Raw8<TO> aux, res, old;
    __device__ __forceinline__ void load(const Epi& e, int64_t m, int64_t n, const TO* D, int64_t ldd) {
        if (e.act == ISEG_ACT_GELU_GRAD || e.act == ISEG_ACT_RELU_GRAD || e.act == ISEG_ACT_MUL_AUX)
            aux.load(reinterpret_cast<const TO*>(e.aux) + m * e.ldaux + n);
        if (e.residual) res.load(reinterpret_cast<const TO*>(e.residual) + m * e.ldr + n);
        if (e.accumulate) old.load(D + m * ldd + n);
    }
};

template <class TO>
__device__ __forceinline__ void epi_finish8(const Epi& e, float* v, const EpiPrefetch<TO>& pf, int64_t m, int64_t n, TO* D, int64_t ldd) {
    constexpr bool FAST = sizeof(TO) == 2;
#pragma unroll
    for (int i = 0; i < 8; ++i) v[i] *= e.alpha;
    if (e.bias) {
        float b[8];
        load8<float>(e.bias + n, b);
#pragma unroll
        for (int i = 0; i < 8; ++i) v[i] += b[i];
    }
    if (e.pre_out && !e.pre_deriv) store8<TO>(reinterpret_cast<TO*>(e.pre_out) + m * e.ldp + n, v);
    if (e.act == ISEG_ACT_RELU) {
#pragma unroll
        for (int i = 0; i < 8; ++i) v[i] = fmaxf(v[i], 0.f);
    } else if (e.act == ISEG_ACT_GELU) {
        if (e.pre_out && e.pre_deriv) {
            float d[8];
#pragma unroll
            for (int i = 0; i < 8; ++i) {
                if (FAST) gelu_sig_both(v[i], v[i], d[i]);
                else {
                    d[i] = gelu_erf_grad(v[i]);
                    v[i] = gelu_erf(v[i]);
                }
            }
            store8<TO>(reinterpret_cast<TO*>(e.pre_out) + m * e.ldp + n, d);
        } else {
#pragma unroll
            for (int i = 0; i < 8; ++i) v[i] = FAST ? gelu_poly(v[i]) : gelu_erf(v[i]);
        }
    } else if (e.act == ISEG_ACT_MUL_AUX) {
#pragma unroll
        for (int i = 0; i < 8; ++i) v[i] *= pf.aux.get(i);
    } else if (e.act == ISEG_ACT_GELU_GRAD) {
#pragma unroll
        for (int i = 0; i < 8; ++i) v[i] *= FAST ? gelu_poly_grad(pf.aux.get(i)) : gelu_erf_grad(pf.aux.get(i));
    } else if (e.act == ISEG_ACT_RELU_GRAD) {
#pragma unroll
        for (int i = 0; i < 8; ++i) v[i] = pf.aux.get(i) > 0.f ? v[i] : 0.f;
    }
    if (e.colscale) {
        float c[8];
        load8<float>(e.colscale + n, c);
#pragma unroll
        for (int i = 0; i < 8; ++i) v[i] *= c[i];
    }
    if (e.rowscale) {
        const float s = e.rowscale[m / e.rows_per_group];
#pragma unroll
        for (int i = 0; i < 8; ++i) v[i] *= s;
    }
    if (e.residual) {
#pragma unroll
        for (int i = 0; i < 8; ++i) v[i] += pf.res.get(i);
    }
    if (e.accumulate) {
#pragma unroll
        for (int i = 0; i < 8; ++i) v[i] += pf.old.get(i);
    }
    store8<TO>(D + m * ldd + n, v);
}

__device__ __forceinline__ int xcd_remap(int b, int nwg) {
    const int q = nwg >> 3, r = nwg & 7, xcd = b & 7;
    const int base = xcd < r ? xcd * (q + 1) : r * (q + 1) + (xcd - r) * q;
    return base + (b >> 3);
}

__device__ __forceinline__ void tile_and_split(int ntiles, int& tile, int& split) {
    if (gridDim.y > 1) {
        const int v = xcd_remap(blockIdx.y * gridDim.x + blockIdx.x, ntiles * gridDim.y);
        tile = v % ntiles;
        split = v / ntiles;
    } else {
        tile = xcd_remap(blockIdx.x, ntiles);
        split = 0;
    }
}

constexpr int KPAD = 8;
constexpr int MNPAD = 8;

typedef __attribute__((address_space(3))) bf16x4* lds_bf16x4_ptr;

template <int ROWS, bool KC, int BK> struct TileGeom {
    static constexpr int stride = KC ? (BK + KPAD) : (ROWS + MNPAD);
    static constexpr int elems = KC ? ROWS * stride : BK * stride;
    static constexpr int chunks = ROWS * BK / 8;
};

template <bool KC>
__device__ __forceinline__ bf16x8 load_chunk(const bf16_t* __restrict__ base, int64_t ld, int64_t r0, int64_t k0, int64_t R,
                                             int64_t Kend, bool vec) {
    bf16x8 v;
#pragma unroll
    for (int i = 0; i < 8; ++i) v[i] = (bf16_t)0.f;
    if (KC) {
        if (r0 >= R || k0 >= Kend) return v;
        const bf16_t* p = base + r0 * ld + k0;
        if (vec && k0 + 8 <= Kend) return *reinterpret_cast<const bf16x8*>(p);
#pragma unroll
        for (int i = 0; i < 8; ++i)
            if (k0 + i < Kend) v[i] = p[i];
    } else {
        if (k0 >= Kend || r0 >= R) return v;
        const bf16_t* p = base + k0 * ld + r0;
        if (vec && r0 + 8 <= R) return *reinterpret_cast<const bf16x8*>(p);
#pragma unroll
        for (int i = 0; i < 8; ++i)
            if (r0 + i < R) v[i] = p[i];
    }
    return v;
}

template <int ROWS, bool KC, int NTHREADS, int BK> struct Stager {
    using G = TileGeom<ROWS, KC, BK>;
    static constexpr int PER_THREAD = (G::chunks + NTHREADS - 1) / NTHREADS;
    bf16x8 regs[PER_THREAD];

    __device__ __forceinline__ static void decode(int c, int& r, int& k) {
        if (KC) {
            r = c / (BK / 8);
            k = (c % (BK / 8)) * 8;
        } else {
            k = c / (ROWS / 8);
            r = (c % (ROWS / 8)) * 8;
        }
    }
    __device__ __forceinline__ void load(const bf16_t* __restrict__ base, int64_t ld, int64_t row0, int64_t k0, int64_t R,
                                         int64_t Kend, bool vec, int tid, bool ones_row = false) {
#pragma unroll
        for (int i = 0; i < PER_THREAD; ++i) {
            const int c = tid + i * NTHREADS;
            if (G::chunks % NTHREADS == 0 || c < G::chunks) {
                int r, k;
                decode(c, r, k);
                regs[i] = load_chunk<KC>(base, ld, row0 + r, k0 + k, R, Kend, vec);
                if (!KC && ones_row && row0 + r == R && k0 + k < Kend) regs[i][0] = (bf16_t)1.0f;
            }
        }
    }
    __device__ __forceinline__ void apply_gelu() {
#pragma unroll
        for (int i = 0; i < PER_THREAD; ++i)
#pragma unroll
            for (int u = 0; u < 8; ++u) regs[i][u] = (bf16_t)gelu_poly((float)regs[i][u]);
    }
    __device__ __forceinline__ void store(bf16_t* lds, int tid) const {
#pragma unroll
        for (int i = 0; i < PER_THREAD; ++i) {
            const int c = tid + i * NTHREADS;
            if (G::chunks % NTHREADS == 0 || c < G::chunks) {
                int r, k;
                decode(c, r, k);
                bf16_t* p = KC ? lds + r * G::stride + k : lds + k * G::stride + r;
                *reinterpret_cast<bf16x8*>(p) = regs[i];
            }
        }
    }
};

template <int ROWS, bool KC, int BK>
__device__ __forceinline__ bf16x8 read_frag(const bf16_t* lds, int r0, int ks, int lane) {
    using G = TileGeom<ROWS, KC, BK>;
    if (KC) {
        return *reinterpret_cast<const bf16x8*>(lds + (r0 + (lane & 15)) * G::stride + 32 * ks + 8 * (lane >> 4));
    } else {
        const int g = lane >> 4, q = (lane >> 2) & 3, p = lane & 3;
        const bf16_t* a0 = lds + (32 * ks + 8 * g + q) * G::stride + r0 + 4 * p;
        const bf16_t* a1 = a0 + 4 * G::stride;
        bf16x4 lo = __builtin_amdgcn_ds_read_tr16_b64_v4bf16((lds_bf16x4_ptr)(a0));
        bf16x4 hi = __builtin_amdgcn_ds_read_tr16_b64_v4bf16((lds_bf16x4_ptr)(a1));
        bf16x8 f;
#pragma unroll
        for (int i = 0; i < 4; ++i) {
            f[i] = lo[i];
            f[4 + i] = hi[i];
        }
        return f;
    }
}

struct IdentityRows {
    __device__ __forceinline__ int64_t operator()(int64_t m) const { return m; }
};

template <int WM, int WN, int FM, int FN, class TO, class RowMap = IdentityRows>
__device__ __forceinline__ void tile_epilogue(f32x4 (&acc)[FM][FN], char* smem, TO* __restrict__ D, int64_t ldd, int64_t M, int64_t N,
                                              int64_t m0, int64_t n0, int wm, int wn, int wid, int lane, float* __restrict__ slabs,
                                              const Epi& epi, bool ones_row, int vecD, int ksplit, const RowMap rowmap = RowMap()) {
    constexpr int TM = FM * 16, TN = FN * 16;
    constexpr int EPI_ROWS = 32;
    constexpr int EPI_STRIDE = TN + 4;
    float* const ew = reinterpret_cast<float*>(smem) + wid * EPI_ROWS * EPI_STRIDE;
    const bool split = slabs != nullptr;
    const int64_t slab_rows = M + (ones_row ? 1 : 0);
    float* const slab = split ? slabs + (int64_t)ksplit * slab_rows * N : nullptr;
    constexpr int PASSES = (TM + EPI_ROWS - 1) / EPI_ROWS;
    constexpr int FPP = EPI_ROWS / 16;
    constexpr int CPR = TN / 8;
#pragma unroll
    for (int ps = 0; ps < PASSES; ++ps) {
#pragma unroll
        for (int fi = 0; fi < FPP; ++fi) {
            const int i = ps * FPP + fi;
            if (i < FM) {
#pragma unroll
                for (int j = 0; j < FN; ++j)
                    *reinterpret_cast<float4*>(ew + (fi * 16 + (lane & 15)) * EPI_STRIDE + j * 16 + (lane >> 4) * 4) =
                        make_float4(acc[i][j][0], acc[i][j][1], acc[i][j][2], acc[i][j][3]);
            }
        }
        __builtin_amdgcn_wave_barrier();
        constexpr int ITERS = (EPI_ROWS * CPR + 63) / 64;
        constexpr int PF = 1;
#pragma unroll
        for (int g0 = 0; g0 < ITERS; g0 += PF) {
            float v[PF][8];
            EpiPrefetch<TO> pf[PF];
            int64_t mm[PF], nn[PF];
            int kind[PF];
#pragma unroll
            for (int q = 0; q < PF; ++q) {
                const int c = lane + (g0 + q) * 64;
                const int rr = c / CPR, cc = (c % CPR) * 8;
                mm[q] = m0 + wm * TM + ps * EPI_ROWS + rr;
                nn[q] = n0 + wn * TN + cc;
                kind[q] = 0;
                if (g0 + q < ITERS && c < EPI_ROWS * CPR && ps * EPI_ROWS + rr < TM && mm[q] < slab_rows && nn[q] < N) {
                    const float* src = ew + rr * EPI_STRIDE + cc;
                    *reinterpret_cast<float4*>(v[q]) = *reinterpret_cast<const float4*>(src);
                    *reinterpret_cast<float4*>(v[q] + 4) = *reinterpret_cast<const float4*>(src + 4);
                    kind[q] = split ? 1 : (mm[q] == M ? 4 : ((vecD && nn[q] + 8 <= N) ? 2 : 3));
                    if (kind[q] == 2 || kind[q] == 3) mm[q] = rowmap(mm[q]);
                    if (kind[q] == 2) pf[q].load(epi, mm[q], nn[q], D, ldd);
                }
            }
#pragma unroll
            for (int q = 0; q < PF; ++q) {
                const int64_t m = mm[q], n = nn[q];
                if (kind[q] == 1) {
                    float* dst = slab + m * N + n;
                    if (n + 8 <= N && (N % 4 == 0)) {
                        *reinterpret_cast<float4*>(dst) = *reinterpret_cast<const float4*>(v[q]);
                        *reinterpret_cast<float4*>(dst + 4) = *reinterpret_cast<const float4*>(v[q] + 4);
                    } else {
                        for (int u = 0; u < 8 && n + u < N; ++u) dst[u] = v[q][u];
                    }
                } else if (kind[q] == 2) {
                    epi_finish8<TO>(epi, v[q], pf[q], m, n, D, ldd);
                } else if (kind[q] == 3) {
                    for (int u = 0; u < 8 && n + u < N; ++u)
                        D[m * ldd + n + u] = from_f32<TO>(epi_apply<TO>(epi, v[q][u], m, n + u, D, ldd));
                } else if (kind[q] == 4) {
                    for (int u = 0; u < 8 && n + u < N; ++u)
                        epi.colsum_out[n + u] = v[q][u] + (epi.colsum_accumulate ? epi.colsum_out[n + u] : 0.f);
                }
            }
        }
        __builtin_amdgcn_wave_barrier();
    }
}

template <int WM, int WN, int FM, int FN, bool AKC, bool BKC, int BK, class TO>
__global__ __launch_bounds__(WM* WN * 64) void gemm_bf16_kernel(const bf16_t* __restrict__ A, int64_t lda,
                                                                 const bf16_t* __restrict__ B, int64_t ldb, TO* __restrict__ D,
                                                                 int64_t ldd, int64_t M, int64_t N, int64_t K, int tiles_n,
                                                                 int ntiles, int64_t k_per_split, float* __restrict__ slabs,
                                                                 Epi epi, int vecA, int vecB, int vecD, int a_act) {
    constexpr int NT = WM * WN * 64;
    constexpr int BM = WM * FM * 16, BN = WN * FN * 16;
    constexpr int TM = FM * 16, TN = FN * 16;
    constexpr int KS = BK / 32;
    using GA = TileGeom<BM, AKC, BK>;
    using GB = TileGeom<BN, BKC, BK>;
    constexpr int STAGE_ELEMS = GA::elems + GB::elems;
    constexpr int EPI_ROWS = 32;
    constexpr int EPI_STRIDE = TN + 4;
    constexpr int EPI_BYTES = WM * WN * EPI_ROWS * EPI_STRIDE * 4;
    constexpr int LDS_BYTES = (STAGE_ELEMS * 2 > EPI_BYTES) ? STAGE_ELEMS * 2 : EPI_BYTES;
    __shared__ __attribute__((aligned(16))) char smem[LDS_BYTES];
    bf16_t* const lds = reinterpret_cast<bf16_t*>(smem);

    const int tid = threadIdx.x, lane = tid & 63, wid = tid >> 6;
    const int wm = wid / WN, wn = wid % WN;
    if (gridDim.z > 1) {
        A += epi.off_a(blockIdx.z);
        B += epi.off_b(blockIdx.z);
        D += epi.off_d(blockIdx.z);
    }

    int t, ksplit;
    tile_and_split(ntiles, t, ksplit);
    const int tile_n = t % tiles_n, tile_m = t / tiles_n;
    const int64_t m0 = (int64_t)tile_m * BM, n0 = (int64_t)tile_n * BN;
    const int64_t kbeg = (int64_t)ksplit * k_per_split;
    const int64_t kend = (kbeg + k_per_split < K) ? kbeg + k_per_split : K;
    const int nk = (int)((kend - kbeg + BK - 1) / BK);

    f32x4 acc[FM][FN];
#pragma unroll
    for (int i = 0; i < FM; ++i)
#pragma unroll
        for (int j = 0; j < FN; ++j) acc[i][j] = f32x4{0.f, 0.f, 0.f, 0.f};

    Stager<BM, AKC, NT, BK> sa;
    Stager<BN, BKC, NT, BK> sb;

    const bool ones_row = !AKC && epi.colsum_out != nullptr;
    sa.load(A, lda, m0, kbeg, M, kend, vecA != 0, tid, ones_row);
    sb.load(B, ldb, n0, kbeg, N, kend, vecB != 0, tid);
    if (a_act == ISEG_ACT_GELU) sa.apply_gelu();
    sa.store(lds, tid);
    sb.store(lds + GA::elems, tid);
    __syncthreads();

    for (int kt = 0; kt < nk; ++kt) {
        const bool more = kt + 1 < nk;
        if (more) {
            const int64_t k0 = kbeg + (int64_t)(kt + 1) * BK;
            sa.load(A, lda, m0, k0, M, kend, vecA != 0, tid, ones_row);
            sb.load(B, ldb, n0, k0, N, kend, vecB != 0, tid);
        }
#pragma unroll
        for (int ks = 0; ks < KS; ++ks) {
            bf16x8 af[FM], bfr[FN];
#pragma unroll
            for (int i = 0; i < FM; ++i) af[i] = read_frag<BM, AKC, BK>(lds, wm * TM + i * 16, ks, lane);
#pragma unroll
            for (int j = 0; j < FN; ++j) bfr[j] = read_frag<BN, BKC, BK>(lds + GA::elems, wn * TN + j * 16, ks, lane);
#pragma unroll
            for (int i = 0; i < FM; ++i)
#pragma unroll
                for (int j = 0; j < FN; ++j)
                    acc[i][j] = __builtin_amdgcn_mfma_f32_16x16x32_bf16(bfr[j], af[i], acc[i][j], 0, 0, 0);
        }
        __syncthreads();
        if (more) {
            if (a_act == ISEG_ACT_GELU) sa.apply_gelu();
            sa.store(lds, tid);
            sb.store(lds + GA::elems, tid);
            __syncthreads();
        }
    }

    tile_epilogue<WM, WN, FM, FN, TO>(acc, smem, D, ldd, M, N, m0, n0, wm, wn, wid, lane, slabs, epi, ones_row, vecD, ksplit);
}

template <int WM, int WN, int FM, int FN, bool AKC, bool BKC, int BK, class TO>
void launch_bf16(const iseg_gemm_args* g, const Epi& epi, int nsplit, int64_t k_per_split, float* slabs, hipStream_t s) {
    constexpr int BM = WM * FM * 16, BN = WN * FN * 16;
    const int tiles_m = (int)ceil_div64(g->M + ((!AKC && epi.colsum_out) ? 1 : 0), BM), tiles_n = (int)ceil_div64(g->N, BN);
    const int ntiles = tiles_m * tiles_n;
    const bf16_t* A = (const bf16_t*)g->A;
    const bf16_t* B = (const bf16_t*)g->B;
    const int vecA = ((uintptr_t)A % 16 == 0) && (g->lda % 8 == 0);
    const int vecB = ((uintptr_t)B % 16 == 0) && (g->ldb % 8 == 0);
    int vecD = ((uintptr_t)g->D % 16 == 0) && (g->ldd % 8 == 0);
    if (g->residual) vecD = vecD && ((uintptr_t)g->residual % 16 == 0) && (g->ldr % 8 == 0);
    if (g->aux) vecD = vecD && ((uintptr_t)g->aux % 16 == 0) && (g->ldaux % 8 == 0);
    if (g->pre_out) vecD = vecD && ((uintptr_t)g->pre_out % 16 == 0) && (g->ldp % 8 == 0);
    if (g->bias) vecD = vecD && ((uintptr_t)g->bias % 16 == 0);
    if (g->colscale) vecD = vecD && ((uintptr_t)g->colscale % 16 == 0);
    const int batch = g->batch > 1 ? g->batch : 1;
    int vA = vecA, vB = vecB, vD = vecD;
    if (batch > 1) {
        vA = vA && g->sa_outer % 8 == 0 && g->sa_inner % 8 == 0;
        vB = vB && g->sb_outer % 8 == 0 && g->sb_inner % 8 == 0;
        vD = vD && g->sd_outer % 8 == 0 && g->sd_inner % 8 == 0;
    }
    dim3 grid(ntiles, nsplit, batch);
    hipLaunchKernelGGL((gemm_bf16_kernel<WM, WN, FM, FN, AKC, BKC, BK, TO>), grid, dim3(WM * WN * 64), 0, s, A, g->lda, B, g->ldb,
                       (TO*)g->D, g->ldd, g->M, g->N, g->K, tiles_n, ntiles, k_per_split, slabs, epi, vA, vB, vD, g->a_act);
}

template <bool AKC, bool BKC, int BK, class TO>
void dispatch_tile(const iseg_gemm_args* g, const Epi& epi, int nsplit, int64_t kps, float* slabs, hipStream_t s) {
    const int64_t N = g->N;
    if (N <= 32) launch_bf16<8, 1, 1, 2, AKC, BKC, BK, TO>(g, epi, nsplit, kps, slabs, s);
    else if (N <= 64) launch_bf16<4, 2, 2, 2, AKC, BKC, BK, TO>(g, epi, nsplit, kps, slabs, s);
    else if (N % 128 != 0 && N % 96 == 0) launch_bf16<4, 2, 2, 3, AKC, BKC, BK, TO>(g, epi, nsplit, kps, slabs, s);
    else launch_bf16<2, 4, 4, 2, AKC, BKC, BK, TO>(g, epi, nsplit, kps, slabs, s);
}

template <bool AKC, bool BKC, class TO>
void dispatch_bk(const iseg_gemm_args* g, const Epi& epi, int nsplit, int64_t kps, float* slabs, hipStream_t s) {
    const int64_t kspan = kps < g->K ? kps : g->K;
    if (AKC && kspan > 64 && kspan <= 96) dispatch_tile<AKC, BKC, 96, TO>(g, epi, nsplit, kps, slabs, s);
    else if (kspan >= 256) dispatch_tile<AKC, BKC, 128, TO>(g, epi, nsplit, kps, slabs, s);
    else dispatch_tile<AKC, BKC, 64, TO>(g, epi, nsplit, kps, slabs, s);
}

void gemm_bf16_nn(const iseg_gemm_args* g, const Epi& epi, int nsplit, int64_t kps, float* slabs, hipStream_t s);
void gemm_bf16_nt(const iseg_gemm_args* g, const Epi& epi, int nsplit, int64_t kps, float* slabs, hipStream_t s);
void gemm_bf16_tn(const iseg_gemm_args* g, const Epi& epi, int nsplit, int64_t kps, float* slabs, hipStream_t s);
int gemm_bf16_tn_pair_split(const iseg_gemm_args* g0, const iseg_gemm_args* g1);
void gemm_bf16_tn_pair(const iseg_gemm_args* g0, float* slabs0, const iseg_gemm_args* g1, float* slabs1, int nsplit, int64_t kps, hipStream_t s);

}
```

### iseg_amd/csrc/gemm_nt.hip

```cpp
#include "gemm_dma.h"

namespace iseg_mm {
void gemm_bf16_nt(const iseg_gemm_args* g, const Epi& epi, int nsplit, int64_t kps, float* slabs, hipStream_t s) {
    if (dma_eligible(g, kps)) {
        if (g->out_dtype == ISEG_BF16) dispatch_dma<bf16_t>(g, epi, nsplit, kps, slabs, s);
        else dispatch_dma<float>(g, epi, nsplit, kps, slabs, s);
        return;
    }
    if (g->out_dtype == ISEG_BF16) dispatch_bk<true, true, bf16_t>(g, epi, nsplit, kps, slabs, s);
    else dispatch_bk<true, true, float>(g, epi, nsplit, kps, slabs, s);
}
}
```

### iseg_amd/functional.py

```python
import os

import torch
from torch.autograd import Function

from . import kernels as K
from . import nn
from . import dist


def _grad(p):
    if p.grad is None:
        p.grad = torch.zeros_like(p.data)
    return p.grad


def _c(t):
    return t if t.is_contiguous() else t.contiguous()


def _rows2d(t):
    C = t.shape[-1]
    if t.is_contiguous():
        return t.reshape(-1, C), C
    per16 = 16 // t.element_size()
# ... 205 lines not shown
    def forward(ctx, x, ln_gamma, ln_beta, eps, W1, b1, W2, b2, rowscale):
        C = x.shape[-1]
        x2 = _c(x).reshape(-1, C)
        M = x2.shape[0]
        rpg = M // rowscale.shape[0] if rowscale is not None else 0
        fw, bw = nn.mlp_tiled(W1, W2, None)
        out, mean, rstd = K.convnext_mlp_fwd_ln(x2, ln_gamma.data, ln_beta.data, eps, fw, b1.data, b2.data, None, rowscale, rpg, x2)
        ctx.params, ctx.rpg = (ln_gamma, ln_beta, W1, b1, W2, b2), rpg
        ctx.save_for_backward(x2, mean, rstd, bw, rowscale)
        return out.reshape(x.shape)

    @staticmethod
    def backward(ctx, dout):
        x2, mean, rstd, bw, rowscale = ctx.saved_tensors
        ln_gamma, ln_beta, W1, b1, W2, b2 = ctx.params
        M, C = x2.shape
        do2 = _c(dout).reshape(M, C)
        ln = (mean, rstd, ln_gamma.data, ln_beta.data)
        dx = None
        if ctx.needs_input_grad[0]:
            dln = K.convnext_mlp_bwd_data_ln(x2, do2, bw, b1.data, ln, _grad(ln_gamma), _grad(ln_beta), rowscale, ctx.rpg)
            dx = K.axpby(do2, dln, 1.0, 1.0, out=dln).reshape(dout.shape)
        else:
            K.convnext_mlp_bwd_data_ln(x2, do2, bw, b1.data, ln, _grad(ln_gamma), _grad(ln_beta), rowscale, ctx.rpg)
        K.convnext_mlp_wgrad(x2, do2, bw, b1.data, W2.data, b2.data, None, _grad(W1), _grad(b1), _grad(W2), _grad(b2), None, rowscale, ctx.rpg, ln=ln)
        dist.grads_ready(ln_gamma, ln_beta, W1, b1, W2, b2)
        return (dx,) + (None,) * 8


def ln_mlp_residual_supported(x, params, drop_path_mask=None):
    ln_gamma, ln_beta, W1, b1, W2, b2 = params
    C = x.shape[-1]
    if any(p is None for p in params) or not K.convnext_mlp_supported(C, x.dtype) or C not in (96, 192):
        return False
    if tuple(W1.shape) != (C, 4 * C) or tuple(W2.shape) != (4 * C, C):
        return False
    if not all(p.requires_grad for p in params) and torch.is_grad_enabled() and (x.requires_grad or any(p.requires_grad for p in params)):
        return False
    rows = x.numel() // C
    return drop_path_mask is None or (rows % drop_path_mask.shape[0] == 0 and (rows // drop_path_mask.shape[0]) % 64 == 0)


def ln_mlp_residual(x, ln_gamma, ln_beta, eps, W1, b1, W2, b2, drop_path_mask=None):
    _check_act_dtype(x)
    if nn.dry_run():
        return _dry(x.shape, x)
    return _LnMlpResidualFn.apply(x, ln_gamma, ln_beta, float(eps), W1, b1, W2, b2, drop_path_mask)


def dense(x, W, b=None, act=K.ACT_NONE, kshape=None):
    _check_act_dtype(x)
    if nn.dry_run():
        return _dry((*x.shape[:-1], kshape[1] if kshape is not None else W.shape[-1]), x)
    return _DenseFn.apply(x, W, b, act, kshape)


def _conv_geometry(H, W, kh, kw, strides, dilation, padding):
    sh, sw = strides
    dh, dw = dilation
    if padding == "same":
        Ho, pt = K.same_pad(H, kh, sh, dh)
        Wo, pl = K.same_pad(W, kw, sw, dw)
    elif padding == "valid":
        Ho = (H - (kh - 1) * dh - 1) // sh + 1
        Wo = (W - (kw - 1) * dw - 1) // sw + 1
        pt = pl = 0
    elif isinstance(padding, tuple):
        (pt, pb), (pl, pr) = padding
        Ho = (H + pt + pb - (kh - 1) * dh - 1) // sh + 1
        Wo = (W + pl + pr - (kw - 1) * dw - 1) // sw + 1
    else:
        raise ValueError(f"padding {padding!r} not supported")
    return Ho, Wo, pt, pl


class _Conv2dFn(Function):

    @staticmethod
    def forward(ctx, x, W, b, strides, dilation, padding, groups):
        kh, kw, Cin_g, Cout = W.shape
        N, H, Wd, Cin = x.shape
        if Cin != Cin_g * groups or Cout % groups != 0:
            raise ValueError(f"Conv2D: kernel {tuple(W.shape)} does not fit {Cin} input channels in {groups} groups")
        Ho, Wo, pt, pl = _conv_geometry(H, Wd, kh, kw, strides, dilation, padding)
        cdt = nn.compute_dtype()
        xc = _c(x)
        geom = K.conv_geom(N, H, Wd, Cin, Cout, kh, kw, strides[0], strides[1], dilation[0], dilation[1], pt, pl, Ho, Wo, groups)
        direct = kh == 1 and kw == 1 and strides == (1, 1) and groups == 1 and xc.dtype == cdt and Cin % 8 == 0
        igemm = (not direct) and xc.dtype == cdt and K.conv2d_igemm_supported(geom, cdt)
        M = N * Ho * Wo
        if direct:
            Wt = _kcontig_kernel(W, xc.reshape(-1, Cin), Cin, Cout)
            if Wt is not None:
                y = K.dense_fwd_t(xc.reshape(-1, Cin), Wt, b.data if b is not None else None)
            else:
                y = torch.empty((M, Cout), dtype=cdt, device=x.device)
                K.gemm(xc.reshape(-1, Cin), nn.w(W).reshape(Cin, Cout), y, M, Cout, Cin, lda=Cin, ldb=Cout, ldd=Cout, a_kcontig=1, b_kcontig=0,
                       bias=(b.data if b is not None else None))
        elif igemm:
            Wt = None
            if K.conv2d_igemm_fwd_kt_supported(geom, cdt):
                Wt = nn.wt(W, (kh * kw * Cin, Cout))
            if Wt is not None:
                y = K.conv2d_igemm_fwd_kt(xc, Wt, b.data if b is not None else None, geom)
            else:
                y = K.conv2d_igemm_fwd(xc, nn.w(W), b.data if b is not None else None, geom)
        else:
            y = torch.empty((M, Cout), dtype=cdt, device=x.device)
            Kd, og = kh * kw * Cin_g, Cout // groups
            keep_col = None
            for g in range(groups):
                col = K.im2col(_group_slice(xc, g, Cin_g, groups), kh, kw, strides[0], strides[1], dilation[0], dilation[1], pt, pl, Ho, Wo, cdt)
                K.gemm(col, nn.w(W).reshape(Kd, Cout)[:, g * og:], y[:, g * og:], M, og, Kd, lda=col.stride(0), ldb=Cout, ldd=Cout, a_kcontig=1,
                       b_kcontig=0, bias=(b.data[g * og:(g + 1) * og] if b is not None else None))
                keep_col = col
            ctx.col = keep_col if (groups == 1 and W.requires_grad and not ctx.needs_input_grad[0] and Kd * keep_col.element_size() <=
                                   Cin * xc.element_size() * strides[0] * strides[1]) else None
        ctx.W, ctx.b = W, b
        ctx.geom, ctx.route = geom, (direct, igemm)
        ctx.x_dtype = x.dtype
        ctx.save_for_backward(xc)
        return y.reshape(N, Ho, Wo, Cout)

    @staticmethod
    def backward(ctx, dy):
        (xc,) = ctx.saved_tensors
        W, b, g_ = ctx.W, ctx.b, ctx.geom
        direct, igemm = ctx.route
        N, H, Wd, Cin, Cout, kh, kw, groups = g_.N, g_.H, g_.W, g_.Cin, g_.Cout, g_.KH, g_.KW, g_.groups
        Ho, Wo, pt, pl = g_.Ho, g_.Wo, g_.pt, g_.pl
        st, di = (g_.sh, g_.sw), (g_.dh, g_.dw)
        Cin_g, og = Cin // groups, Cout // groups
        Kd = kh * kw * Cin_g
        cdt = nn.compute_dtype()
        M = N * Ho * Wo
        dy2 = _c(dy).reshape(M, Cout)
        if b is not None and b.requires_grad:
            K.colsum(dy2, Cout, 0, 1, M, Cout, _grad(b), accumulate=True)
        need_dx = ctx.needs_input_grad[0]
        dx = None
        if direct:
            if W.requires_grad:
                K.gemm(xc.reshape(-1, Cin), dy2, _grad(W).reshape(Cin, Cout), Cin, Cout, M, lda=Cin, ldb=Cout, ldd=Cout, a_kcontig=0, b_kcontig=0,
                       accumulate=True)
            if need_dx:
                dx = K.dense_dgrad(dy2, nn.w(W).reshape(Cin, Cout)).reshape(N, H, Wd, Cin)
        elif igemm:
            dy4 = dy2.reshape(N, Ho, Wo, Cout)
            if W.requires_grad:
                K.conv2d_igemm_bwd_weight(xc, dy4, _grad(W), g_, accumulate=True)
            patchify = (kh, kw) == st
            if need_dx and (st == (1, 1) or (di == (1, 1) and st[0] * st[1] <= 16 and not patchify)):
                dx = K.conv2d_igemm_bwd_data(dy4, nn.w(W), g_)
            elif need_dx:
                ldc = (Kd + 7) // 8 * 8
                dx = torch.empty((N, H, Wd, Cin), dtype=cdt, device=dy.device) if groups > 1 else None
                for g in range(groups):
                    dcol = torch.empty((M, ldc), dtype=cdt, device=dy.device)
                    K.gemm(dy2[:, g * og:], nn.w(W).reshape(Kd, Cout)[:, g * og:], dcol, M, Kd, og, lda=Cout, ldb=Cout, ldd=ldc, a_kcontig=1,
                           b_kcontig=1)
                    dxg = K.col2im(dcol, N, H, Wd, Cin_g, kh, kw, st[0], st[1], di[0], di[1], pt, pl, Ho, Wo)
                    if groups == 1:
                        dx = dxg
                    else:
                        K.copy2d(dxg.reshape(-1, Cin_g), Cin_g, dx.reshape(-1, Cin)[:, g * Cin_g:], Cin, N * H * Wd, Cin_g)
        else:
            if need_dx:
                dx = torch.empty((N, H, Wd, Cin), dtype=cdt, device=dy.device)
            ldc = (Kd + 7) // 8 * 8
            for g in range(groups):
                dyg = dy2[:, g * og:]
                if W.requires_grad:
                    col = getattr(ctx, "col", None)
                    if col is None:
                        col = K.im2col(_group_slice(xc, g, Cin_g, groups), kh, kw, st[0], st[1], di[0], di[1], pt, pl, Ho, Wo, cdt)
                    K.gemm(col, dyg, _grad(W).reshape(Kd, Cout)[:, g * og:], Kd, og, M, lda=col.stride(0), ldb=Cout, ldd=Cout, a_kcontig=0,
                           b_kcontig=0, accumulate=True)
                    del col
                if need_dx:
                    dcol = torch.empty((M, ldc), dtype=cdt, device=dy.device)
                    K.gemm(dyg, nn.w(W).reshape(Kd, Cout)[:, g * og:], dcol, M, Kd, og, lda=Cout, ldb=Cout, ldd=ldc, a_kcontig=1, b_kcontig=1)
                    dxg = K.col2im(dcol, N, H, Wd, Cin_g, kh, kw, st[0], st[1], di[0], di[1], pt, pl, Ho, Wo)
                    if groups == 1:
                        dx = dxg
                    else:
                        K.copy2d(dxg.reshape(-1, Cin_g), Cin_g, dx.reshape(-1, Cin)[:, g * Cin_g:], Cin, N * H * Wd, Cin_g)
        if dx is not None and dx.dtype != ctx.x_dtype:
            dx = K.cast(dx, ctx.x_dtype)
        dist.grads_ready(W, b)
        return dx, None, None, None, None, None, None


def _group_slice(xc, g, Cin_g, groups):
    if groups == 1:
        return xc
    N, H, W, Cin = xc.shape
    out = torch.empty((N, H, W, Cin_g), dtype=xc.dtype, device=xc.device)
    K.copy2d(xc.reshape(-1, Cin)[:, g * Cin_g:], Cin, out.reshape(-1, Cin_g), Cin_g, N * H * W, Cin_g)
    return out


def conv2d(x, W, b=None, strides=(1, 1), dilation=(1, 1), padding="same", groups=1):
    if nn.dry_run():
        Ho, Wo, _, _ = _conv_geometry(x.shape[1], x.shape[2], W.shape[0], W.shape[1], tuple(strides), tuple(dilation), padding)
        return _dry((x.shape[0], Ho, Wo, W.shape[-1]), x, nn.compute_dtype())
    return _Conv2dFn.apply(x, W, b, tuple(strides), tuple(dilation), padding, int(groups))


class _DWConvFn(Function):
    @staticmethod
    def forward(ctx, x, W, b, dil):
        Kk, C = W.shape[0], W.shape[2]
        pad = (Kk - 1) * dil // 2
        xc = _c(x)
        y = K.dwconv2d(xc, W.data.reshape(Kk * Kk, C), b.data if b is not None else None, Kk, dil, pad, pad)
        ctx.W, ctx.b, ctx.dil, ctx.pad = W, b, dil, pad
        ctx.save_for_backward(xc)
        return y

    @staticmethod
    def backward(ctx, dy):
        (xc,) = ctx.saved_tensors
        W, b, dil, pad = ctx.W, ctx.b, ctx.dil, ctx.pad
        Kk, C = W.shape[0], W.shape[2]
        dyc = _c(dy)
        if W.requires_grad:
            K.dwconv2d_bwd_weight(xc, dyc, _grad(W).reshape(Kk * Kk, C), _grad(b) if b is not None else None, Kk, dil, pad, pad)
        dx = None
        if ctx.needs_input_grad[0]:
            padb = (Kk - 1) * dil - pad
            dx = K.dwconv2d(dyc, W.data.reshape(Kk * Kk, C), None, Kk, dil, padb, padb, flip=True)
        dist.grads_ready(W, b)
        return dx, None, None, None


class _DWConvStridedFn(Function):

    @staticmethod
    def forward(ctx, x, W, b, dil, stride):
        Kk, C = W.shape[0], W.shape[2]
        xc = _c(x)
        y = K.dwconv2d_strided(xc, W.data.reshape(Kk * Kk, C), b.data if b is not None else None, Kk, stride, dil)
        ctx.W, ctx.b, ctx.dil, ctx.stride = W, b, dil, stride
        ctx.save_for_backward(xc)
        return y

    @staticmethod
    def backward(ctx, dy):
        (xc,) = ctx.saved_tensors
        W, b, dil, stride = ctx.W, ctx.b, ctx.dil, ctx.stride
        Kk, C = W.shape[0], W.shape[2]
        dyc = _c(dy)
        if W.requires_grad:
            K.dwconv2d_strided_bwd_weight(xc, dyc, _grad(W).reshape(Kk * Kk, C), _grad(b) if b is not None else None, Kk, stride, dil)
        dx = None
        if ctx.needs_input_grad[0]:
            dx = K.dwconv2d_strided_bwd_data(dyc, W.data.reshape(Kk * Kk, C), Kk, stride, dil, xc.shape[1], xc.shape[2])
        dist.grads_ready(W, b)
        return dx, None, None, None, None


def depthwise_conv2d(x, W, b=None, dilation=1, strides=1):
    _check_act_dtype(x)
    s = int(strides)
    if s == 1:
        if nn.dry_run():
            return _dry(x.shape, x)
        return _DWConvFn.apply(x, W, b, int(dilation))
    N, H, Wd, C = x.shape
    if nn.dry_run():
        return _dry((N, -(-H // s), -(-Wd // s), C), x)
    return _DWConvStridedFn.apply(x, W, b, int(dilation), s)


class _LayerNormFn(Function):
    @staticmethod
    def forward(ctx, x, gamma, beta, eps):
        C = x.shape[-1]
        x2 = _c(x).reshape(-1, C)
        y, mean, rstd = K.layernorm_fwd(x2, gamma.data, beta.data, eps)
        ctx.gamma, ctx.beta = gamma, beta
        ctx.save_for_backward(x2, mean, rstd)
        return y.reshape(x.shape)

    @staticmethod
    def backward(ctx, dy):
        x2, mean, rstd = ctx.saved_tensors
        C = x2.shape[-1]
        dx = K.layernorm_bwd(_c(dy).reshape(-1, C), x2, ctx.gamma.data, mean, rstd, _grad(ctx.gamma), _grad(ctx.beta))
        dist.grads_ready(ctx.gamma, ctx.beta)
        return dx.reshape(dy.shape), None, None, None


class _LayerNormPostFn(Function):

    @staticmethod
    def forward(ctx, x, gamma, beta, eps, colscale, rowscale, residual):
        C = x.shape[-1]
        x2 = _c(x).reshape(-1, C)
        rpg = x2.shape[0] // rowscale.shape[0] if rowscale is not None else 0
        r2 = _c(residual).reshape(-1, C) if residual is not None else None
        y, mean, rstd = K.layernorm_post_fwd(x2, gamma.data, beta.data, eps, colscale.data if colscale is not None else None, rowscale, rpg, r2)
        ctx.params, ctx.rpg = (gamma, beta, colscale), rpg
        ctx.save_for_backward(x2, mean, rstd, rowscale)
        return y.reshape(x.shape)

# ... 2173 lines not shown
```

### iseg_amd/kernels.py

```python
import contextlib
import ctypes as C

import torch

from . import _hip
from ._hip import F32, BF16, ACT_NONE, ACT_RELU, ACT_GELU, ACT_GELU_GRAD, ACT_RELU_GRAD, ACT_MUL_AUX, ACT_SIGMOID, ACT_SWISH, GemmArgs

_DT = {torch.float32: F32, torch.bfloat16: BF16}


def dt(t):
    try:
        return _DT[t.dtype if isinstance(t, torch.Tensor) else t]
    except KeyError:
        raise TypeError(f"iseg_amd kernels support float32 and bfloat16 storage, got {t.dtype if isinstance(t, torch.Tensor) else t}")


def ptr(t):
    return None if t is None else t.data_ptr()


_DEVICE_INDEX = [None]


def stream():
    idx = _DEVICE_INDEX[0]
    if idx is None:
        idx = _DEVICE_INDEX[0] = torch.cuda.current_device()
    return torch._C._cuda_getCurrentRawStream(idx)


def _require_cuda(*ts):
    for t in ts:
        if t is not None and not t.is_cuda:
            raise _hip.HipCallError("iseg_amd kernels need device tensors (cuda:N); there is no CPU path")


_WS = {}


def workspace(nbytes, device):
    if nbytes <= 0:
        return None, 0
    key = (device.index if device.index is not None else torch.cuda.current_device(), stream())
    buf = _WS.get(key)
    if buf is None or buf.numel() < nbytes:
        size = int(nbytes * 1.25) + 1024
        if torch.cuda.is_current_stream_capturing():
            if buf is not None:
                raise _hip.HipCallError("workspace growth during hipGraph capture; run one eager warm-up step first")
            size = max([size] + [b.numel() for (d, _), b in _WS.items() if d == key[0]])
        buf = torch.empty(size, dtype=torch.uint8, device=device)
        _WS[key] = buf
    return buf, buf.numel()


KERNEL_TIMER = [None]


class KernelTimer:

    def __init__(self, only=None, every=1):
        self.records = {}
        self.seen = {}
        self._cur = None
        self.only = only
        self._only = None if only is None else (set(only) if isinstance(only, (set, list, frozenset)) else {only})
        self.every = max(1, int(every))

    def begin(self, key):
        if self._only is not None and key not in self._only:
            self._cur = None
            return
        n = self.seen.get(key, 0)
        self.seen[key] = n + 1
        if n % self.every:
            self._cur = None
            return
        e0 = torch.cuda.Event(enable_timing=True)
        e0.record()
        self._cur = (key, e0)

    def end(self):
        if self._cur is None:
            return
        key, e0 = self._cur
        e1 = torch.cuda.Event(enable_timing=True)
        e1.record()
        self.records.setdefault(key, []).append((e0, e1))

    def report(self):
        torch.cuda.synchronize()
        out = {}
        for key, pairs in self.records.items():
            ms = [a.elapsed_time(b) for a, b in pairs]
            out[key] = (sum(ms) / len(ms) * 1e-3, self.seen.get(key, len(ms)))
        return out


def gemm(A, B, D, M, N, K, *, lda, ldb, ldd, a_kcontig, b_kcontig, bias=None, colscale=None, rowscale=None,
         rows_per_group=0, residual=None, ldr=0, aux=None, ldaux=0, pre_out=None, ldp=0, act=ACT_NONE, alpha=1.0,
         accumulate=False, split_k=0, a_act=ACT_NONE, colsum_out=None, colsum_accumulate=False, batch=1, batch_inner=1,
         sa=(0, 0), sb=(0, 0), sd=(0, 0), pre_deriv=False, b_group=None):
    _require_cuda(A, B, D)
    if A.dtype != B.dtype:
        raise TypeError(f"gemm operands differ in dtype: {A.dtype} vs {B.dtype}")
    g = GemmArgs()
    g.A, g.lda, g.a_kcontig = ptr(A), lda, int(a_kcontig)
    g.B, g.ldb, g.b_kcontig = ptr(B), ldb, int(b_kcontig)
    g.D, g.ldd = ptr(D), ldd
    g.M, g.N, g.K = M, N, K
    g.in_dtype, g.out_dtype = dt(A), dt(D)
    g.bias, g.colscale, g.rowscale, g.rows_per_group = ptr(bias), ptr(colscale), ptr(rowscale), rows_per_group
    g.residual, g.ldr = ptr(residual), ldr
    g.aux, g.ldaux = ptr(aux), ldaux
    g.pre_out, g.ldp = ptr(pre_out), ldp
    g.act, g.alpha, g.accumulate, g.split_k, g.a_act = act, alpha, int(accumulate), split_k, a_act
    g.colsum_out, g.colsum_accumulate = ptr(colsum_out), int(colsum_accumulate)
    g.batch, g.batch_inner = int(batch), int(batch_inner)
    g.pre_deriv = int(bool(pre_deriv))
    g.b_group_rows, g.b_group_stride = (int(b_group[0]), int(b_group[1])) if b_group is not None else (0, 0)
    (g.sa_outer, g.sa_inner), (g.sb_outer, g.sb_inner), (g.sd_outer, g.sd_inner) = sa, sb, sd
    for t in (residual, aux, pre_out):
        if t is not None and t.dtype != D.dtype:
            raise TypeError("gemm residual/aux/pre_out must have the output dtype")
    for t in (bias, colscale, rowscale):
        if t is not None and t.dtype != torch.float32:
            raise TypeError("gemm bias/colscale/rowscale must be float32")
    L = _hip.lib()
    need = L.iseg_gemm_workspace_bytes(C.byref(g))
    ws, wsb = workspace(need, A.device)
    g.defer_reduce = 1 if need > 0 else 0
    timer = KERNEL_TIMER[0]
    if timer is not None:
        timer.begin(("gemm", int(a_kcontig), int(b_kcontig), int(M), int(N), int(K), int(act), pre_out is not None, residual is not None,
                     aux is not None, A.dtype, D.dtype, need > 0, int(L.iseg_gemm_variant(C.byref(g)))) + ((int(batch),) if batch > 1 else ()))
    _hip.check(L.iseg_gemm(C.byref(g), ptr(ws), wsb, stream()), "iseg_gemm")
    if timer is not None:
        timer.end()
    if need > 0:
        _hip.check(L.iseg_gemm_reduce(C.byref(g), ptr(ws), wsb, stream()), "iseg_gemm_reduce")
    return D


def dense_fwd(x2d, W, bias=None, *, act=ACT_NONE, out=None, ldd=None, out_dtype=None, pre_out=None, colscale=None,
              rowscale=None, rows_per_group=0, residual=None, a_act=ACT_NONE, pre_deriv=False):
    M, K = x2d.shape
    N = W.shape[1]
    if out is None:
        out = torch.empty((M, N), dtype=out_dtype or x2d.dtype, device=x2d.device)
    return gemm(x2d, W, out, M, N, K, lda=x2d.stride(0), ldb=W.stride(0), ldd=ldd or out.stride(0), a_kcontig=1, b_kcontig=0,
                bias=bias, act=act, pre_out=pre_out, ldp=(pre_out.stride(0) if pre_out is not None else 0), colscale=colscale,
                rowscale=rowscale, rows_per_group=rows_per_group, residual=residual,
                ldr=(residual.stride(0) if residual is not None else 0), a_act=a_act, pre_deriv=pre_deriv)


def dense_fwd_t(x2d, Wt, bias=None, *, act=ACT_NONE, out=None, pre_out=None, colscale=None, rowscale=None, rows_per_group=0, residual=None,
                pre_deriv=False):
    M, K = x2d.shape
    N = Wt.shape[0]
    if out is None:
        out = torch.empty((M, N), dtype=x2d.dtype, device=x2d.device)
    return gemm(x2d, Wt, out, M, N, K, lda=x2d.stride(0), ldb=Wt.stride(0), ldd=out.stride(0), a_kcontig=1, b_kcontig=1, bias=bias, act=act,
                pre_out=pre_out, ldp=(pre_out.stride(0) if pre_out is not None else 0), colscale=colscale, rowscale=rowscale,
                rows_per_group=rows_per_group, residual=residual, ldr=(residual.stride(0) if residual is not None else 0), pre_deriv=pre_deriv)


def dense_dgrad(dy2d, W, *, out=None, act=ACT_NONE, aux=None, rowscale=None, rows_per_group=0, residual=None, accumulate=False):
    M, N = dy2d.shape
    K = W.shape[0]
    if out is None:
        out = torch.empty((M, K), dtype=dy2d.dtype, device=dy2d.device)
    return gemm(dy2d, W, out, M, K, N, lda=dy2d.stride(0), ldb=W.stride(0), ldd=out.stride(0), a_kcontig=1, b_kcontig=1, act=act,
                aux=aux, ldaux=(aux.stride(0) if aux is not None else 0), rowscale=rowscale, rows_per_group=rows_per_group,
                residual=residual, ldr=(residual.stride(0) if residual is not None else 0), accumulate=accumulate)


def wgrad_can_fuse_bias(x2d):
    k = x2d.shape[1]
    return x2d.dtype == torch.bfloat16 and k % 8 == 0 and (k % 128 != 0 or k >= 384)


def dense_wgrad(x2d, dy2d, out, *, accumulate=True, alpha=1.0, a_act=ACT_NONE, bias_grad=None):
    M, K = x2d.shape
    N = dy2d.shape[1]
    fuse = bias_grad is not None and wgrad_can_fuse_bias(x2d)
    if bias_grad is not None and not fuse:
        colsum(dy2d, dy2d.stride(0), 0, 1, M, N, bias_grad, accumulate=accumulate)
    return gemm(x2d, dy2d, out, K, N, M, lda=x2d.stride(0), ldb=dy2d.stride(0), ldd=out.stride(0), a_kcontig=0, b_kcontig=0,
                accumulate=accumulate, alpha=alpha, a_act=a_act, colsum_out=(bias_grad if fuse else None),
                colsum_accumulate=accumulate)


def dense_wgrad_slabs(x2d, dy2d):
    M, K = x2d.shape
    N = dy2d.shape[1]
    if not wgrad_can_fuse_bias(x2d) or N % 4 != 0 or x2d.dtype != torch.bfloat16:
        return None
    _require_cuda(x2d, dy2d)
    g = GemmArgs()
    dummy = torch.empty(1, dtype=torch.float32, device=x2d.device)
    g.A, g.lda, g.a_kcontig = ptr(x2d), x2d.stride(0), 0
    g.B, g.ldb, g.b_kcontig = ptr(dy2d), dy2d.stride(0), 0
    g.D, g.ldd = ptr(dummy), N
    g.M, g.N, g.K = K, N, M
    g.in_dtype, g.out_dtype = dt(x2d), 0
    g.alpha, g.accumulate = 1.0, 0
    g.colsum_out, g.colsum_accumulate = ptr(dummy), 0
    g.batch, g.batch_inner = 1, 1
    L = _hip.lib()
    need = L.iseg_gemm_workspace_bytes(C.byref(g))
    if need == 0:
        return None
    eff = int(L.iseg_gemm_slabs(C.byref(g)))
    slabs = torch.empty(need // 4, dtype=torch.float32, device=x2d.device)
    g.defer_reduce = 1
    timer = KERNEL_TIMER[0]
    if timer is not None:
        timer.begin(("gemm", 0, 0, int(K), int(N), int(M), 0, False, False, False, x2d.dtype, torch.float32, True, int(L.iseg_gemm_variant(C.byref(g)))))
    _hip.check(L.iseg_gemm(C.byref(g), ptr(slabs), need, stream()), "iseg_gemm")
    if timer is not None:
        timer.end()
    return slabs, int(eff)


def dense_wgrad_pair(g2d, dbr2d, x2d, dh2d, dW1, db1, accumulate=True, defer_second=False):
    rows, K4 = g2d.shape
    Cc = dbr2d.shape[1]
    if not (wgrad_can_fuse_bias(g2d) and wgrad_can_fuse_bias(x2d)) or Cc % 4 != 0:
        return None
    _require_cuda(g2d, dbr2d, x2d, dh2d, dW1)
    dummy = torch.empty(1, dtype=torch.float32, device=g2d.device)

    def args(a, b, out, ldd, bias, acc):
        g = GemmArgs()
        g.A, g.lda, g.a_kcontig = ptr(a), a.stride(0), 0
        g.B, g.ldb, g.b_kcontig = ptr(b), b.stride(0), 0
        g.D, g.ldd = ptr(out), ldd
        g.M, g.N, g.K = a.shape[1], b.shape[1], rows
        g.in_dtype, g.out_dtype = dt(a), 0
        g.alpha, g.accumulate = 1.0, int(acc)
        g.colsum_out, g.colsum_accumulate = ptr(bias), int(acc)
        g.batch, g.batch_inner = 1, 1
        g.defer_reduce = 1
        return g

    g0 = args(g2d, dbr2d, dummy, Cc, dummy, False)
    g1 = args(x2d, dh2d, dW1, dW1.stride(0), db1, accumulate)
    L = _hip.lib()
    s = int(L.iseg_gemm_tn_pair_splits(C.byref(g0), C.byref(g1)))
    if s <= 1:
        return None
    g0.split_k = g1.split_k = s
    need0, need1 = L.iseg_gemm_workspace_bytes(C.byref(g0)), L.iseg_gemm_workspace_bytes(C.byref(g1))
    eff = int(L.iseg_gemm_slabs(C.byref(g0)))
    slabs0 = torch.empty(need0 // 4, dtype=torch.float32, device=g2d.device)
    n2 = (x2d.shape[1] + 1) * dh2d.shape[1]
    n0 = x2d.shape[1] * dh2d.shape[1]
    defer_second = bool(defer_second and dW1.stride(0) == dh2d.shape[1] and n2 % 4 == 0 and n0 % 4 == 0 and dW1.is_contiguous() and db1 is not None)
    if defer_second:
        ws1 = torch.empty(need1 // 4, dtype=torch.float32, device=g2d.device)
        wsb1 = need1
    else:
        ws1, wsb1 = workspace(need1, g2d.device)
    timer = KERNEL_TIMER[0]
    if timer is not None:
        timer.begin(("gemm", 0, 0, int(K4), int(Cc), int(rows), 0, False, False, False, g2d.dtype, torch.float32, True, 9))
    _hip.check(L.iseg_gemm_tn_pair(C.byref(g0), ptr(slabs0), need0, C.byref(g1), ptr(ws1), wsb1, stream()), "iseg_gemm_tn_pair")
    if timer is not None:
        timer.end()
    if defer_second:
        eff1 = int(L.iseg_gemm_slabs(C.byref(g1)))
        return slabs0, eff, (ws1, eff1, n2, dW1, db1, n0, bool(accumulate))
    _hip.check(L.iseg_gemm_reduce(C.byref(g1), ptr(ws1), wsb1, stream()), "iseg_gemm_reduce")
    return slabs0, eff
# ... 1355 lines not shown
```

Before: 1964.

## Scatter patchify-conv input gradient directly into NHWC layout from GEMM epilogue

For a patchify convolution (kernel equals stride, no padding), the data-gradient GEMM now writes its output straight into the NHWC dx tensor through a patch row map in the epilogue. This replaces the earlier path that wrote a column buffer and then ran a col2im or rearrangement step. The cost removed is the extra buffer write, its re-read and the scatter kernel. In exchange, the epilogue index math gets more complex (integer div/mod per store), and split-K is forced off for this GEMM, which may hurt occupancy.

```diff
diff --git a/include/iseg_hip.h b/include/iseg_hip.h
--- a/include/iseg_hip.h
+++ b/include/iseg_hip.h
@@ -67,6 +67,7 @@
     int64_t sa_outer, sa_inner, sb_outer, sb_inner, sd_outer, sd_inner;
     int pre_deriv;
     int64_t b_group_rows, b_group_stride;
+    int patch_wo, patch_run, patch_kh;
 } iseg_gemm_args;
 
 int iseg_gemm_splits(const iseg_gemm_args* args_h);
diff --git a/iseg_amd/_hip.py b/iseg_amd/_hip.py
--- a/iseg_amd/_hip.py
+++ b/iseg_amd/_hip.py
@@ -35,6 +35,7 @@
         ("pre_deriv", C.c_int),
         ("b_group_rows", C.c_int64),
         ("b_group_stride", C.c_int64),
+        ("patch_wo", C.c_int), ("patch_run", C.c_int), ("patch_kh", C.c_int),
     ]
 
 
diff --git a/iseg_amd/csrc/conv_igemm.hip b/iseg_amd/csrc/conv_igemm.hip
--- a/iseg_amd/csrc/conv_igemm.hip
+++ b/iseg_amd/csrc/conv_igemm.hip
@@ -173,6 +173,7 @@
     D += grp * d_group_stride;
     if (slabs) slabs += grp * slab_group_stride;
     if (epi.bias) epi.bias += grp * N;
+    epi.patch_wo = 0;
 
     int t, ksplit;
     int tw = p.kw, tap0 = 0, tsh = p.kw, tsw = 1;
diff --git a/iseg_amd/csrc/conv_igemm_dma.h b/iseg_amd/csrc/conv_igemm_dma.h
--- a/iseg_amd/csrc/conv_igemm_dma.h
+++ b/iseg_amd/csrc/conv_igemm_dma.h
@@ -21,6 +21,7 @@
 
     const int tid = threadIdx.x, lane = tid & 63, wid = tid >> 6;
     const int wm = wid / WN, wn = wid % WN;
+    epi.patch_wo = 0;
     int t, ksplit;
     tile_and_split(ntiles, t, ksplit);
     const int64_t m0 = (int64_t)(t / tiles_n) * BM, n0 = (int64_t)(t % tiles_n) * BN;
diff --git a/iseg_amd/csrc/gemm.hip b/iseg_amd/csrc/gemm.hip
--- a/iseg_amd/csrc/gemm.hip
+++ b/iseg_amd/csrc/gemm.hip
@@ -24,11 +24,11 @@
 void gemm_log(const iseg_gemm_args* g, int nsplit) {
     static GemmCensus census;
     char buf[256];
-    snprintf(buf, sizeof buf, "%s %s->%s M=%lld N=%lld K=%lld batch=%d split=%d form=%d act=%d a_act=%d%s%s%s%s%s%s%s%s%s%s", g->a_kcontig ? (g->b_kcontig ? "NT" : "NN") : (g->b_kcontig ? "TT" : "TN"),
+    snprintf(buf, sizeof buf, "%s %s->%s M=%lld N=%lld K=%lld batch=%d split=%d form=%d act=%d a_act=%d%s%s%s%s%s%s%s%s%s%s%s", g->a_kcontig ? (g->b_kcontig ? "NT" : "NN") : (g->b_kcontig ? "TT" : "TN"),
              g->in_dtype == ISEG_BF16 ? "bf16" : "f32", g->out_dtype == ISEG_BF16 ? "bf16" : "f32", (long long)g->M, (long long)g->N, (long long)g->K,
              g->batch > 1 ? g->batch : 1, nsplit, iseg_gemm_variant(g), g->act, g->a_act, g->bias ? " bias" : "", g->residual ? " residual" : "",
              g->aux ? " aux" : "", g->pre_out ? " pre_out" : "", g->colsum_out ? " colsum" : "", g->colscale ? " colscale" : "", g->rowscale ? " rowscale" : "",
-             g->pre_deriv ? " pre_deriv" : "", g->accumulate ? " accumulate" : "", g->alpha != 1.f ? " alpha" : "");
+             g->pre_deriv ? " pre_deriv" : "", g->accumulate ? " accumulate" : "", g->alpha != 1.f ? " alpha" : "", g->patch_wo > 0 ? " patch" : "");
     std::lock_guard<std::mutex> lock(census.mu);
     ++census.seen[buf];
 }
@@ -56,6 +56,7 @@
     __shared__ float sB[TK][TB + 1];
     const int tid = threadIdx.x;
     const int tx = tid & 15, ty = tid >> 4;
+    epi.patch_wo = 0;
     if (gridDim.z > 1) {
         A += epi.off_a(blockIdx.z);
         B += epi.off_b(blockIdx.z);
@@ -108,6 +109,7 @@
 __global__ void splitk_reduce_kernel(const float* __restrict__ slabs, int nsplit, TO* __restrict__ D, int64_t ldd, int64_t M,
                                      int64_t N, Epi epi, int64_t slab_rows) {
     const int64_t total = slab_rows * N;
+    epi.patch_wo = 0;
     for (int64_t i = blockIdx.x * (int64_t)blockDim.x + threadIdx.x; i < total; i += (int64_t)gridDim.x * blockDim.x) {
         float s = 0.f;
         for (int z = 0; z < nsplit; ++z) s += slabs[(int64_t)z * total + i];
@@ -119,6 +121,7 @@
 
 int choose_split(const iseg_gemm_args* g, int tile) {
     if (g->split_k > 0) return g->split_k;
+    if (g->patch_wo > 0) return 1;
     if (const int form = iseg_mm::dma_tn_form(g)) {
         const int s = iseg_mm::dma_tn_split(g, form);
         if (s > 1) return s;
@@ -178,9 +181,9 @@
     ISEG_REQUIRE(!g->pre_deriv || (g->act == ISEG_ACT_GELU && g->pre_out), "iseg_gemm: pre_deriv needs act = GELU and pre_out");
     ISEG_REQUIRE(g->a_act == ISEG_ACT_NONE || g->a_act == ISEG_ACT_GELU, "iseg_gemm: a_act must be NONE or GELU");
     Epi epi{g->bias, g->colscale, g->rowscale, g->rows_per_group, g->residual, g->ldr, g->aux, g->ldaux, g->pre_out, g->ldp,
-            g->act, g->alpha, g->accumulate, g->colsum_out, g->colsum_accumulate,
+            g->act, g->alpha, g->accumulate, g->patch_wo, g->colsum_out, g->colsum_accumulate,
             g->batch_inner > 0 ? g->batch_inner : 1, g->sa_outer, g->sa_inner, g->sb_outer, g->sb_inner, g->sd_outer, g->sd_inner,
-            g->pre_deriv, g->b_group_rows, g->b_group_stride};
+            g->pre_deriv, g->patch_run, g->b_group_rows, g->b_group_stride};
     const int batch = g->batch > 1 ? g->batch : 1;
     if (batch > 1) {
         ISEG_REQUIRE(batch <= 65535, "iseg_gemm: batch %d exceeds the grid z limit (65535)", batch);
@@ -193,6 +196,17 @@
               g->b_group_stride % 8 == 0 && iseg_mm::dma_eligible(g, g->K))) {
             iseg_set_error("iseg_gemm: B per row group needs the LDS-DMA path (bf16, K-contiguous operands, K %% 64 == 0, aligned) with "
                            "b_group_rows %% 256 == 0, no split and no batch");
+            return ISEG_ERR_UNSUPPORTED;
+        }
+    }
+    if (g->patch_wo > 0) {
+        const bool plain = !g->bias && !g->colscale && !g->rowscale && !g->residual && !g->aux && !g->pre_out && !g->colsum_out &&
+                           g->act == ISEG_ACT_NONE && g->a_act == ISEG_ACT_NONE && g->alpha == 1.f && !g->accumulate;
+        if (!(g->in_dtype == ISEG_BF16 && g->out_dtype == ISEG_BF16 && g->a_kcontig && g->b_kcontig && plain && batch == 1 && g->split_k <= 1 &&
+              g->patch_run > 0 && g->patch_kh > 0 && g->patch_run % 8 == 0 && g->N == (int64_t)g->patch_kh * g->patch_run &&
+              g->M % g->patch_wo == 0 && g->M < (1ll << 31) && g->ldd == g->N && (uintptr_t)g->D % 16 == 0)) {
+            iseg_set_error("iseg_gemm: the patch row map needs bf16 storage, both operands K-contiguous, a plain epilogue, N == patch_kh * patch_run, "
+                           "patch_run %% 8 == 0, M %% patch_wo == 0, ldd == N, a 16-byte aligned D, no split and no batch");
             return ISEG_ERR_UNSUPPORTED;
         }
     }
@@ -296,9 +310,9 @@
     const int64_t kps = ceil_div64(ceil_div64(g->K, nsplit), 128) * 128;
     const int eff_split = (int)ceil_div64(g->K, kps);
     Epi epi{g->bias, g->colscale, g->rowscale, g->rows_per_group, g->residual, g->ldr, g->aux, g->ldaux, g->pre_out, g->ldp,
-            g->act, g->alpha, g->accumulate, g->colsum_out, g->colsum_accumulate,
+            g->act, g->alpha, g->accumulate, g->patch_wo, g->colsum_out, g->colsum_accumulate,
             g->batch_inner > 0 ? g->batch_inner : 1, g->sa_outer, g->sa_inner, g->sb_outer, g->sb_inner, g->sd_outer, g->sd_inner,
-            g->pre_deriv, g->b_group_rows, g->b_group_stride};
+            g->pre_deriv, g->patch_run, g->b_group_rows, g->b_group_stride};
     const int batch = g->batch > 1 ? g->batch : 1;
     if (batch > 1) {
         ISEG_REQUIRE(batch <= 65535, "iseg_gemm: batch %d exceeds the grid z limit (65535)", batch);
diff --git a/iseg_amd/csrc/gemm_dma.h b/iseg_amd/csrc/gemm_dma.h
--- a/iseg_amd/csrc/gemm_dma.h
+++ b/iseg_amd/csrc/gemm_dma.h
@@ -9,7 +9,7 @@
 
 __device__ __forceinline__ int b_key(int row) { return (row & 3) | (((row >> 3) & 1) << 2); }
 
-enum { EK_ANY = 0, EK_GELU_DERIV = 1, EK_MUL_AUX = 2, EK_BIAS_RESIDUAL = 3, EK_PLAIN = 4, EK_BIAS = 5 };
+enum { EK_ANY = 0, EK_GELU_DERIV = 1, EK_MUL_AUX = 2, EK_BIAS_RESIDUAL = 3, EK_PLAIN = 4, EK_BIAS = 5, EK_PLAIN_PATCH = 6 };
 
 template <int EK> __device__ __forceinline__ Epi epi_known(Epi e) {
     if (EK == EK_GELU_DERIV) {
@@ -28,7 +28,7 @@
         e.colscale = nullptr;
         e.accumulate = 0;
         e.alpha = 1.f;
-    } else if (EK == EK_PLAIN) {
+    } else if (EK == EK_PLAIN || EK == EK_PLAIN_PATCH) {
         e.act = ISEG_ACT_NONE;
         e.bias = nullptr;
         e.aux = nullptr;
@@ -54,6 +54,7 @@
         e.accumulate = 0;
         e.alpha = 1.f;
     }
+    if (EK != EK_PLAIN_PATCH) e.patch_wo = 0;
     return e;
 }
 
@@ -62,6 +63,7 @@
 constexpr int dma_min_k = 32;
 
 inline int epi_kind(const Epi& e, const float* slabs) {
+    if (e.patch_wo > 0) return EK_PLAIN_PATCH;
     if (slabs || e.alpha != 1.f || e.accumulate) return EK_ANY;
     if (e.act == ISEG_ACT_GELU && e.pre_out && e.pre_deriv && e.bias && !e.residual && !e.aux && !e.colscale) return EK_GELU_DERIV;
     if (e.act == ISEG_ACT_MUL_AUX && e.aux && !e.bias && !e.pre_out && !e.residual && !e.colscale) return EK_MUL_AUX;
@@ -338,6 +340,12 @@
 
 template <int WM, int WN, int NS, class TO, int FN, int BKS = 64, int FM = 4>
 void launch_dma_kinds(const iseg_gemm_args* g, const Epi& epi, int nsplit, int64_t kps, float* slabs, hipStream_t s) {
+    if constexpr (sizeof(TO) == 2) {
+        if (epi.patch_wo > 0) {
+            launch_dma<WM, WN, NS, TO, FN, EK_PLAIN_PATCH, BKS, FM>(g, epi, nsplit, kps, slabs, s);
+            return;
+        }
+    }
     if (sizeof(TO) == 2) {
         switch (epi_kind(epi, slabs)) {
             case EK_GELU_DERIV: launch_dma<WM, WN, NS, TO, FN, EK_GELU_DERIV, BKS, FM>(g, epi, nsplit, kps, slabs, s); return;
@@ -351,18 +359,29 @@
     launch_dma<WM, WN, NS, TO, FN, EK_ANY, BKS, FM>(g, epi, nsplit, kps, slabs, s);
 }
 
+template <int WM, int WN, int NS, class TO>
+void launch_dma_any(const iseg_gemm_args* g, const Epi& epi, int nsplit, int64_t kps, float* slabs, hipStream_t s) {
+    if constexpr (sizeof(TO) == 2) {
+        if (epi.patch_wo > 0) {
+            launch_dma<WM, WN, NS, TO, 4, EK_PLAIN_PATCH>(g, epi, nsplit, kps, slabs, s);
+            return;
+        }
+    }
+    launch_dma<WM, WN, NS, TO>(g, epi, nsplit, kps, slabs, s);
+}
+
 int dma_bk32();
 
 template <class TO>
 void dispatch_dma(const iseg_gemm_args* g, const Epi& epi, int nsplit, int64_t kps, float* slabs, hipStream_t s) {
     switch (dma_form(g, nsplit)) {
-        case 1: launch_dma<2, 1, 4, TO>(g, epi, nsplit, kps, slabs, s); break;
+        case 1: launch_dma_any<2, 1, 4, TO>(g, epi, nsplit, kps, slabs, s); break;
         case 2:
             if (dma_bk32() && (dma_bk32() == 2 || g->K <= 512) && g->K % 32 == 0 && g->K >= 96 && (kps == g->K || kps % 64 == 0) && sizeof(TO) == 2)
                 launch_dma_kinds<4, 2, 3, TO, 4, 32>(g, epi, nsplit, kps, slabs, s);
             else launch_dma_kinds<4, 2, 3, TO, 4>(g, epi, nsplit, kps, slabs, s);
             break;
-        case 3: launch_dma<2, 2, 2, TO>(g, epi, nsplit, kps, slabs, s); break;
+        case 3: launch_dma_any<2, 2, 2, TO>(g, epi, nsplit, kps, slabs, s); break;
         case 6: launch_dma_kinds<4, 2, 2, TO, 6>(g, epi, nsplit, kps, slabs, s); break;
         case 9: launch_dma_kinds<4, 2, 3, TO, 6, 64, 1>(g, epi, nsplit, kps, slabs, s); break;
         case 8: launch_dma_kinds<4, 2, 3, TO, 6, 64, 2>(g, epi, nsplit, kps, slabs, s); break;
diff --git a/iseg_amd/csrc/gemm_impl.h b/iseg_amd/csrc/gemm_impl.h
--- a/iseg_amd/csrc/gemm_impl.h
+++ b/iseg_amd/csrc/gemm_impl.h
@@ -18,16 +18,26 @@
     int act;
     float alpha;
     int accumulate;
+    int patch_wo;
     float* colsum_out;
     int colsum_accumulate;
     int batch_inner;
     int64_t sa_outer, sa_inner, sb_outer, sb_inner, sd_outer, sd_inner;
     int pre_deriv;
+    int patch_run;
     int64_t b_group_rows, b_group_stride;
     __device__ __forceinline__ int64_t off_a(int z) const { return (z / batch_inner) * sa_outer + (z % batch_inner) * sa_inner; }
     __device__ __forceinline__ int64_t off_b(int z) const { return (z / batch_inner) * sb_outer + (z % batch_inner) * sb_inner; }
     __device__ __forceinline__ int64_t off_d(int z) const { return (z / batch_inner) * sd_outer + (z % batch_inner) * sd_inner; }
-};
+    __device__ __forceinline__ int64_t d_at(int64_t m, int64_t n, int64_t ldd) const {
+        if (patch_wo == 0) return m * ldd + n;
+        const unsigned wo = (unsigned)patch_wo, run = (unsigned)patch_run;
+        const unsigned mq = (unsigned)m / wo, mr = (unsigned)m - mq * wo, nq = (unsigned)n / run, nr = (unsigned)n - nq * run;
+        return ((int64_t)mq * ldd + (int64_t)nq * run) * wo + (int64_t)mr * run + nr;
+    }
+};
+
+static_assert(sizeof(Epi) == 184, "Epi: the patch row map must stay inside the alignment holes");
 
 template <class TO>
 __device__ __forceinline__ float epi_apply(const Epi& e, float acc, int64_t m, int64_t n, const TO* D, int64_t ldd) {
@@ -42,7 +52,7 @@
     if (e.colscale) v *= e.colscale[n];
     if (e.rowscale) v *= e.rowscale[m / e.rows_per_group];
     if (e.residual) v += to_f32(reinterpret_cast<const TO*>(e.residual)[m * e.ldr + n]);
-    if (e.accumulate) v += to_f32(D[m * ldd + n]);
+    if (e.accumulate) v += to_f32(D[e.d_at(m, n, ldd)]);
     return v;
 }
 
@@ -110,13 +120,14 @@
 #pragma unroll
         for (int i = 0; i < 8; ++i) v[i] += r[i];
     }
+    TO* const d = D + e.d_at(m, n, ldd);
     if (e.accumulate) {
         float r[8];
-        load8<TO>(D + m * ldd + n, r);
+        load8<TO>(d, r);
 #pragma unroll
         for (int i = 0; i < 8; ++i) v[i] += r[i];
     }
-    store8<TO>(D + m * ldd + n, v);
+    store8<TO>(d, v);
 }
 
 template <class T> struct Raw8;
@@ -142,7 +153,7 @@
         if (e.act == ISEG_ACT_GELU_GRAD || e.act == ISEG_ACT_RELU_GRAD || e.act == ISEG_ACT_MUL_AUX)
             aux.load(reinterpret_cast<const TO*>(e.aux) + m * e.ldaux + n);
         if (e.residual) res.load(reinterpret_cast<const TO*>(e.residual) + m * e.ldr + n);
-        if (e.accumulate) old.load(D + m * ldd + n);
+        if (e.accumulate) old.load(D + e.d_at(m, n, ldd));
     }
 };
 
@@ -206,7 +217,7 @@
 #pragma unroll
         for (int i = 0; i < 8; ++i) v[i] += pf.old.get(i);
     }
-    store8<TO>(D + m * ldd + n, v);
+    store8<TO>(D + e.d_at(m, n, ldd), v);
 }
 
 __device__ __forceinline__ int xcd_remap(int b, int nwg) {
@@ -399,7 +410,7 @@
                     epi_finish8<TO>(epi, v[q], pf[q], m, n, D, ldd);
                 } else if (kind[q] == 3) {
                     for (int u = 0; u < 8 && n + u < N; ++u)
-                        D[m * ldd + n + u] = from_f32<TO>(epi_apply<TO>(epi, v[q][u], m, n + u, D, ldd));
+                        D[epi.d_at(m, n + u, ldd)] = from_f32<TO>(epi_apply<TO>(epi, v[q][u], m, n + u, D, ldd));
                 } else if (kind[q] == 4) {
                     for (int u = 0; u < 8 && n + u < N; ++u)
                         epi.colsum_out[n + u] = v[q][u] + (epi.colsum_accumulate ? epi.colsum_out[n + u] : 0.f);
@@ -410,7 +421,7 @@
     }
 }
 
-template <int WM, int WN, int FM, int FN, bool AKC, bool BKC, int BK, class TO>
+template <int WM, int WN, int FM, int FN, bool AKC, bool BKC, int BK, class TO, bool PATCH = false>
 __global__ __launch_bounds__(WM* WN * 64) void gemm_bf16_kernel(const bf16_t* __restrict__ A, int64_t lda,
                                                                  const bf16_t* __restrict__ B, int64_t ldb, TO* __restrict__ D,
                                                                  int64_t ldd, int64_t M, int64_t N, int64_t K, int tiles_n,
@@ -432,6 +443,7 @@
 
     const int tid = threadIdx.x, lane = tid & 63, wid = tid >> 6;
     const int wm = wid / WN, wn = wid % WN;
+    if (!PATCH) epi.patch_wo = 0;
     if (gridDim.z > 1) {
         A += epi.off_a(blockIdx.z);
         B += epi.off_b(blockIdx.z);
@@ -495,7 +507,7 @@
     tile_epilogue<WM, WN, FM, FN, TO>(acc, smem, D, ldd, M, N, m0, n0, wm, wn, wid, lane, slabs, epi, ones_row, vecD, ksplit);
 }
 
-template <int WM, int WN, int FM, int FN, bool AKC, bool BKC, int BK, class TO>
+template <int WM, int WN, int FM, int FN, bool AKC, bool BKC, int BK, class TO, bool PATCH = false>
 void launch_bf16(const iseg_gemm_args* g, const Epi& epi, int nsplit, int64_t k_per_split, float* slabs, hipStream_t s) {
     constexpr int BM = WM * FM * 16, BN = WN * FN * 16;
     const int tiles_m = (int)ceil_div64(g->M + ((!AKC && epi.colsum_out) ? 1 : 0), BM), tiles_n = (int)ceil_div64(g->N, BN);
@@ -518,25 +530,25 @@
         vD = vD && g->sd_outer % 8 == 0 && g->sd_inner % 8 == 0;
     }
     dim3 grid(ntiles, nsplit, batch);
-    hipLaunchKernelGGL((gemm_bf16_kernel<WM, WN, FM, FN, AKC, BKC, BK, TO>), grid, dim3(WM * WN * 64), 0, s, A, g->lda, B, g->ldb,
+    hipLaunchKernelGGL((gemm_bf16_kernel<WM, WN, FM, FN, AKC, BKC, BK, TO, PATCH>), grid, dim3(WM * WN * 64), 0, s, A, g->lda, B, g->ldb,
                        (TO*)g->D, g->ldd, g->M, g->N, g->K, tiles_n, ntiles, k_per_split, slabs, epi, vA, vB, vD, g->a_act);
 }
 
-template <bool AKC, bool BKC, int BK, class TO>
+template <bool AKC, bool BKC, int BK, class TO, bool PATCH = false>
 void dispatch_tile(const iseg_gemm_args* g, const Epi& epi, int nsplit, int64_t kps, float* slabs, hipStream_t s) {
     const int64_t N = g->N;
-    if (N <= 32) launch_bf16<8, 1, 1, 2, AKC, BKC, BK, TO>(g, epi, nsplit, kps, slabs, s);
-    else if (N <= 64) launch_bf16<4, 2, 2, 2, AKC, BKC, BK, TO>(g, epi, nsplit, kps, slabs, s);
-    else if (N % 128 != 0 && N % 96 == 0) launch_bf16<4, 2, 2, 3, AKC, BKC, BK, TO>(g, epi, nsplit, kps, slabs, s);
-    else launch_bf16<2, 4, 4, 2, AKC, BKC, BK, TO>(g, epi, nsplit, kps, slabs, s);
-}
-
-template <bool AKC, bool BKC, class TO>
+    if (N <= 32) launch_bf16<8, 1, 1, 2, AKC, BKC, BK, TO, PATCH>(g, epi, nsplit, kps, slabs, s);
+    else if (N <= 64) launch_bf16<4, 2, 2, 2, AKC, BKC, BK, TO, PATCH>(g, epi, nsplit, kps, slabs, s);
+    else if (N % 128 != 0 && N % 96 == 0) launch_bf16<4, 2, 2, 3, AKC, BKC, BK, TO, PATCH>(g, epi, nsplit, kps, slabs, s);
+    else launch_bf16<2, 4, 4, 2, AKC, BKC, BK, TO, PATCH>(g, epi, nsplit, kps, slabs, s);
+}
+
+template <bool AKC, bool BKC, class TO, bool PATCH = false>
 void dispatch_bk(const iseg_gemm_args* g, const Epi& epi, int nsplit, int64_t kps, float* slabs, hipStream_t s) {
     const int64_t kspan = kps < g->K ? kps : g->K;
-    if (AKC && kspan > 64 && kspan <= 96) dispatch_tile<AKC, BKC, 96, TO>(g, epi, nsplit, kps, slabs, s);
-    else if (kspan >= 256) dispatch_tile<AKC, BKC, 128, TO>(g, epi, nsplit, kps, slabs, s);
-    else dispatch_tile<AKC, BKC, 64, TO>(g, epi, nsplit, kps, slabs, s);
+    if (AKC && kspan > 64 && kspan <= 96) dispatch_tile<AKC, BKC, 96, TO, PATCH>(g, epi, nsplit, kps, slabs, s);
+    else if (kspan >= 256) dispatch_tile<AKC, BKC, 128, TO, PATCH>(g, epi, nsplit, kps, slabs, s);
+    else dispatch_tile<AKC, BKC, 64, TO, PATCH>(g, epi, nsplit, kps, slabs, s);
 }
 
 void gemm_bf16_nn(const iseg_gemm_args* g, const Epi& epi, int nsplit, int64_t kps, float* slabs, hipStream_t s);
diff --git a/iseg_amd/csrc/gemm_nt.hip b/iseg_amd/csrc/gemm_nt.hip
--- a/iseg_amd/csrc/gemm_nt.hip
+++ b/iseg_amd/csrc/gemm_nt.hip
@@ -7,7 +7,8 @@
         else dispatch_dma<float>(g, epi, nsplit, kps, slabs, s);
         return;
     }
-    if (g->out_dtype == ISEG_BF16) dispatch_bk<true, true, bf16_t>(g, epi, nsplit, kps, slabs, s);
+    if (epi.patch_wo > 0) dispatch_bk<true, true, bf16_t, true>(g, epi, nsplit, kps, slabs, s);
+    else if (g->out_dtype == ISEG_BF16) dispatch_bk<true, true, bf16_t>(g, epi, nsplit, kps, slabs, s);
     else dispatch_bk<true, true, float>(g, epi, nsplit, kps, slabs, s);
 }
 }
diff --git a/iseg_amd/functional.py b/iseg_amd/functional.py
--- a/iseg_amd/functional.py
+++ b/iseg_amd/functional.py
@@ -381,6 +381,11 @@
             patchify = (kh, kw) == st
             if need_dx and (st == (1, 1) or (di == (1, 1) and st[0] * st[1] <= 16 and not patchify)):
                 dx = K.conv2d_igemm_bwd_data(dy4, nn.w(W), g_)
+            elif (need_dx and patchify and cdt == torch.bfloat16 and groups == 1 and di == (1, 1) and (pt, pl) == (0, 0) and
+                  (H, Wd) == (Ho * kh, Wo * kw) and (kw * Cin) % 8 == 0):
+                dx = torch.empty((N, H, Wd, Cin), dtype=cdt, device=dy.device)
+                K.gemm(dy2, nn.w(W).reshape(Kd, Cout), dx, M, Kd, Cout, lda=Cout, ldb=Cout, ldd=Kd, a_kcontig=1, b_kcontig=1,
+                       patch=(Wo, kw * Cin, kh))
             elif need_dx:
                 ldc = (Kd + 7) // 8 * 8
                 dx = torch.empty((N, H, Wd, Cin), dtype=cdt, device=dy.device) if groups > 1 else None
diff --git a/iseg_amd/kernels.py b/iseg_amd/kernels.py
--- a/iseg_amd/kernels.py
+++ b/iseg_amd/kernels.py
@@ -101,7 +101,7 @@
 def gemm(A, B, D, M, N, K, *, lda, ldb, ldd, a_kcontig, b_kcontig, bias=None, colscale=None, rowscale=None,
          rows_per_group=0, residual=None, ldr=0, aux=None, ldaux=0, pre_out=None, ldp=0, act=ACT_NONE, alpha=1.0,
          accumulate=False, split_k=0, a_act=ACT_NONE, colsum_out=None, colsum_accumulate=False, batch=1, batch_inner=1,
-         sa=(0, 0), sb=(0, 0), sd=(0, 0), pre_deriv=False, b_group=None):
+         sa=(0, 0), sb=(0, 0), sd=(0, 0), pre_deriv=False, b_group=None, patch=None):
     _require_cuda(A, B, D)
     if A.dtype != B.dtype:
         raise TypeError(f"gemm operands differ in dtype: {A.dtype} vs {B.dtype}")
@@ -121,6 +121,7 @@
     g.pre_deriv = int(bool(pre_deriv))
     g.b_group_rows, g.b_group_stride = (int(b_group[0]), int(b_group[1])) if b_group is not None else (0, 0)
     (g.sa_outer, g.sa_inner), (g.sb_outer, g.sb_inner), (g.sd_outer, g.sd_inner) = sa, sb, sd
+    g.patch_wo, g.patch_run, g.patch_kh = (int(patch[0]), int(patch[1]), int(patch[2])) if patch is not None else (0, 0, 0)
     for t in (residual, aux, pre_out):
         if t is not None and t.dtype != D.dtype:
             raise TypeError("gemm residual/aux/pre_out must have the output dtype")
```

Result: no change. 1977 (median of 6 runs) (+0.6%).
